# locuslab/lcp-physics

Hardware: NVIDIA H100
Metric: LCP solves/sec (LCPFunction fwd+bwd, batch=4096 x 64 contacts, fp32) (higher is better)
Workload: dtype f32 I/O and iterates; the condensed n x n KKT matrix is formed, factored and solved in f64

## Files before the change

### lcp_physics_b200/csrc/lcp_cond_kernels.cu

```cuda
#include "lcp_cond_launch.h"

namespace lcpb200 {
namespace cnd {

template <>
cudaError_t launch_cond_forward_t<LCP_T, LCP_NS>(const CFwdArgs<LCP_T>& a, int grid, cudaStream_t st) {
  if (a.prof) cond_forward_kernel<LCP_T, LCP_NS, true><<<grid, NT, a.P.smem_bytes, st>>>(a);
  else cond_forward_kernel<LCP_T, LCP_NS, false><<<grid, NT, a.P.smem_bytes, st>>>(a);
  return cudaGetLastError();
}

template <>
cudaError_t launch_cond_backward_t<LCP_T, LCP_NS>(const CBwdArgs<LCP_T>& a, int grid, cudaStream_t st) {
  if (a.prof) cond_backward_kernel<LCP_T, LCP_NS, true><<<grid, NT, a.P.smem_bytes, st>>>(a);
  else cond_backward_kernel<LCP_T, LCP_NS, false><<<grid, NT, a.P.smem_bytes, st>>>(a);
  return cudaGetLastError();
}

template <>
cudaError_t configure_cond_t<LCP_T, LCP_NS>(int smem_bytes, int dyn_max, int* occ) {
  cudaError_t e;
  const void* fns[4] = {(const void*)cond_forward_kernel<LCP_T, LCP_NS, false>, (const void*)cond_backward_kernel<LCP_T, LCP_NS, false>,
                        (const void*)cond_forward_kernel<LCP_T, LCP_NS, true>, (const void*)cond_backward_kernel<LCP_T, LCP_NS, true>};
  for (const void* f : fns)
    if ((e = cudaFuncSetAttribute(f, cudaFuncAttributeMaxDynamicSharedMemorySize, dyn_max)) != cudaSuccess) return e;
  int of = 0, ob = 0;
  if ((e = cudaOccupancyMaxActiveBlocksPerMultiprocessor(&of, fns[0], NT, smem_bytes)) != cudaSuccess) return e;
  if ((e = cudaOccupancyMaxActiveBlocksPerMultiprocessor(&ob, fns[1], NT, smem_bytes)) != cudaSuccess) return e;
  *occ = of < ob ? of : ob;
  return cudaSuccess;
}

}
}
```

### lcp_physics_b200/csrc/lcp_cond_launch.h

```cpp
#pragma once
#include <cuda_runtime.h>
#include "lcp_condensed.cuh"

namespace lcpb200 {
namespace cnd {

template <typename T, int NS> cudaError_t launch_cond_forward_t(const CFwdArgs<T>& a, int grid, cudaStream_t st);
template <typename T, int NS> cudaError_t launch_cond_backward_t(const CBwdArgs<T>& a, int grid, cudaStream_t st);
template <typename T, int NS> cudaError_t configure_cond_t(int smem_bytes, int dyn_max, int* occ);

}
}
```

### lcp_physics_b200/csrc/lcp_condensed.cuh

```cuda
#pragma once
#include "lcp_device.cuh"

namespace lcpb200 {
namespace cnd {

constexpr int NT = 256;
constexpr int UC = 8;
constexpr int CSMAX = 6;
constexpr int KS = 8;
constexpr int LMAX = 16;
constexpr int LU_BW = 2;
constexpr int MISC_BAND_LU = 4;
constexpr int CFLAG_DENSE_LU = 4;
constexpr int STATUS_UNSUPPORTED = -100;

struct CPlan {
  int ok;
  int n, m, e, N, NP, NS;
  int pcap;
  int wcap;
  int smem_bytes;
  int ctas_per_sm;
  int flags;
  int sbytes;
  int o_K, o_W, o_scr, o_bx, o_rdiag, o_Fd, o_Gd, o_As, o_x, o_rx, o_dx, o_qd, o_y, o_ry, o_dy,
      o_s, o_z, o_d, o_rz, o_ds, o_dz, o_rs2, o_red, o_rows, o_posof, o_clist, o_ccols, o_ncols, o_clcnt, o_misc;
};

__host__ __device__ inline size_t al16(size_t x) { return (x + 15) & ~(size_t)15; }
__host__ __device__ inline size_t scratch_bytes(int n, int m, int tsize) {
  return al16((size_t)2 * KS * m * 2) + al16((size_t)2 * KS * m * tsize) + al16((size_t)5 * m * 4) +
         al16((size_t)CSMAX * m * 2) + al16((size_t)8 * m * 4) + al16((size_t)LMAX * n * 2) + al16((size_t)n * 4) + 64;
}

inline size_t carve_plan(CPlan& P, int tsize) {
  size_t o = 0;
  const int n = P.n, m = P.m, e = P.e, NP = P.NP, pcap = P.pcap, wcap = P.wcap;
#define CND_TAKE(field, bytes) do { P.field = (int)o; o += al16((size_t)(bytes)); } while (0)
  size_t kb = (size_t)NP * NP * 8;
  if (scratch_bytes(n, m, tsize) > kb) kb = scratch_bytes(n, m, tsize);
  if ((size_t)8 * NP * 8 > kb) kb = (size_t)8 * NP * 8;
  { const size_t qn = (NP + 31) / 32, sl = (size_t)(NP / qn) * qn * qn * 32 * 8; if (sl > kb) kb = sl; }
  CND_TAKE(o_K, kb);
  CND_TAKE(o_W, (size_t)wcap * 8);
  CND_TAKE(o_scr, (size_t)pcap * 8);
  CND_TAKE(o_bx, (size_t)NP * 8);
  CND_TAKE(o_rdiag, (size_t)NP * 8);
  CND_TAKE(o_Fd, (size_t)wcap * tsize);
  CND_TAKE(o_Gd, (size_t)UC * pcap * tsize);
  CND_TAKE(o_As, (size_t)e * n * tsize);
  CND_TAKE(o_x, n * tsize); CND_TAKE(o_rx, n * tsize); CND_TAKE(o_dx, n * tsize); CND_TAKE(o_qd, n * tsize);
  CND_TAKE(o_y, e * tsize); CND_TAKE(o_ry, e * tsize); CND_TAKE(o_dy, e * tsize);
  CND_TAKE(o_s, m * tsize); CND_TAKE(o_z, m * tsize); CND_TAKE(o_d, m * tsize); CND_TAKE(o_rz, m * tsize);
  CND_TAKE(o_ds, m * tsize); CND_TAKE(o_dz, m * tsize); CND_TAKE(o_rs2, m * tsize);
  CND_TAKE(o_red, 192 * tsize);
  CND_TAKE(o_rows, pcap * 2);
  CND_TAKE(o_posof, m * 2);
  CND_TAKE(o_clist, LMAX * n * 2);
  CND_TAKE(o_ccols, UC * pcap);
  CND_TAKE(o_ncols, pcap);
  CND_TAKE(o_clcnt, n);
  CND_TAKE(o_misc, 16 * 4);
#undef CND_TAKE
  P.sbytes = 16 + (P.o_x - P.o_Fd) + (P.o_y - P.o_qd) + (P.o_misc - P.o_rows);
  return o;
}

extern __shared__ __align__(16) unsigned char cnd_smem[];

template <typename T>
struct CSmem {
  const CPlan& P;
  __device__ __forceinline__ explicit CSmem(const CPlan& p) : P(p) {}
#define CND_ACC(name, type) __device__ __forceinline__ type* name() const { return reinterpret_cast<type*>(cnd_smem + P.o_##name); }
  CND_ACC(K, double) CND_ACC(W, double) CND_ACC(scr, double) CND_ACC(bx, double) CND_ACC(rdiag, double)
  CND_ACC(Fd, T) CND_ACC(Gd, T) CND_ACC(As, T)
  CND_ACC(x, T) CND_ACC(rx, T) CND_ACC(dx, T) CND_ACC(qd, T) CND_ACC(y, T) CND_ACC(ry, T) CND_ACC(dy, T)
  CND_ACC(s, T) CND_ACC(z, T) CND_ACC(d, T) CND_ACC(rz, T) CND_ACC(ds, T) CND_ACC(dz, T) CND_ACC(rs2, T)
  CND_ACC(red, T)
  CND_ACC(rows, unsigned short) CND_ACC(posof, unsigned short) CND_ACC(clist, unsigned short)
  CND_ACC(ccols, unsigned char) CND_ACC(ncols, unsigned char) CND_ACC(clcnt, unsigned char)
  CND_ACC(misc, int)
#undef CND_ACC
};

struct Struct {
  int ncomp, cs;
  int sh;
  int m;
};

enum { CPH_STRUCT = 0, CPH_WINV, CPH_ASSEMBLE, CPH_LU, CPH_SOLVE_RHS, CPH_SOLVE_TRI, CPH_SOLVE_POST, CPH_RESID,
       CPH_STEP, CPH_GRADS, CPH_COUNT };
template <bool ON>
struct Prof {
  long long* p;
  long long t;
  __device__ __forceinline__ explicit Prof(long long* p_) : p(p_), t(0) {}
  __device__ __forceinline__ void start() { if (threadIdx.x == 0) t = clock64(); }
  __device__ __forceinline__ void lap(int ph) {
    if (threadIdx.x == 0) {
      const long long n = clock64();
      atomicAdd(reinterpret_cast<unsigned long long*>(p + ph), (unsigned long long)(n - t));
      t = n;
    }
  }
};
template <>
struct Prof<false> {
  __device__ __forceinline__ explicit Prof(long long*) {}
  __device__ __forceinline__ void start() {}
  __device__ __forceinline__ void lap(int) {}
};

template <typename T>
__device__ __forceinline__ int scan_rows(const T* __restrict__ A, int rows, int cols, T* vals, unsigned short* idx,
                                         int* cnt) {
  constexpr int CH = 8, RP = (sizeof(T) == 8) ? 2 : 4;
  const int lane = threadIdx.x & 31, warp = threadIdx.x >> 5, nw = NT >> 5;
  int bad = 0;
  if (cols <= 32 * CH) {
    for (int r0 = warp * RP; r0 < rows; r0 += nw * RP) {
      T v[RP][CH];
#pragma unroll
      for (int rr = 0; rr < RP; ++rr) {
        const T* row = A + (size_t)min(r0 + rr, rows - 1) * cols;
#pragma unroll
        for (int q = 0; q < CH; ++q) { const int j = q * 32 + lane; v[rr][q] = j < cols ? row[j] : T(0); }
      }
#pragma unroll
      for (int rr = 0; rr < RP; ++rr) {
        const int r = r0 + rr;
        if (r >= rows) break;
        int c = 0;
#pragma unroll
        for (int q = 0; q < CH; ++q) {
          const bool nz = v[rr][q] != T(0);
          const unsigned mask = __ballot_sync(FULL, nz);
          const int pos = c + __popc(mask & ((1u << lane) - 1u));
          if (nz && pos < KS) { vals[pos * rows + r] = v[rr][q]; idx[pos * rows + r] = (unsigned short)(q * 32 + lane); }
          c += __popc(mask);
        }
        if (c > KS) bad = 1;
        if (lane == 0) cnt[r] = c;
      }
    }
    return bad;
  }
  for (int r = warp; r < rows; r += nw) {
    const T* row = A + (size_t)r * cols;
    int c = 0;
    for (int j0 = 0; j0 < cols; j0 += 32 * CH) {
      T v[CH];
#pragma unroll
      for (int q = 0; q < CH; ++q) { const int j = j0 + q * 32 + lane; v[q] = j < cols ? row[j] : T(0); }
#pragma unroll
      for (int q = 0; q < CH; ++q) {
        const bool nz = v[q] != T(0);
        const unsigned mask = __ballot_sync(FULL, nz);
        const int pos = c + __popc(mask & ((1u << lane) - 1u));
        if (nz && pos < KS) { vals[pos * rows + r] = v[q]; idx[pos * rows + r] = (unsigned short)(j0 + q * 32 + lane); }
        c += __popc(mask);
      }
    }
    if (c > KS) bad = 1;
    if (lane == 0) cnt[r] = c;
  }
  return bad;
}

__device__ __forceinline__ void prefetch_l2(const void* p, size_t bytes) {
  const char* c = reinterpret_cast<const char*>(p);
  for (size_t o = (size_t)threadIdx.x * 128; o < bytes; o += (size_t)NT * 128)
    asm volatile("prefetch.global.L2 [%0];" ::"l"(c + o));
}

template <typename T>
__device__ __noinline__ bool build_structure(const CPlan& P, CSmem<T>& S, Struct& st, const T* __restrict__ Q,
                                             const T* __restrict__ G, const T* __restrict__ A,
                                             const T* __restrict__ F, int* singular) {
  const int n = P.n, m = P.m, e = P.e, tid = threadIdx.x, lane = tid & 31, warp = tid >> 5, pcap = P.pcap;
  prefetch_l2(F, (size_t)m * m * sizeof(T));
  prefetch_l2(G, (size_t)m * n * sizeof(T));
  prefetch_l2(Q, (size_t)n * n * sizeof(T));
  char* sb = reinterpret_cast<char*>(S.K());
  unsigned short* Fi = reinterpret_cast<unsigned short*>(sb);
  unsigned short* Gi = Fi + (size_t)KS * m;
  size_t o = al16((size_t)2 * KS * m * 2);
  T* Fv = reinterpret_cast<T*>(sb + o);
  T* Gv = Fv + (size_t)KS * m;
  o += al16((size_t)2 * KS * m * sizeof(T));
  int* Fcnt = reinterpret_cast<int*>(sb + o);
  int* Gcnt = Fcnt + m;
  int* label = Gcnt + m;
  int* cidx = label + m;
  int* memcnt = cidx + m;
  o += al16((size_t)5 * m * 4);
  unsigned short* memb = reinterpret_cast<unsigned short*>(sb + o);
  o += al16((size_t)CSMAX * m * 2);
  unsigned* cmap = reinterpret_cast<unsigned*>(sb + o);
  o += al16((size_t)8 * m * 4);
  unsigned short* cl_tmp = reinterpret_cast<unsigned short*>(sb + o);
  o += al16((size_t)LMAX * n * 2);
  int* cl_cnt = reinterpret_cast<int*>(sb + o);
  int* flags = S.misc();

  if (tid < 16) flags[tid] = 0;
  int bad = 0;
  for (int t = tid; t < n * n; t += NT) {
    const int i = t / n, j = t - i * n;
    const T q = Q[t];
    if (i == j) {
      S.qd()[i] = q;
      if (!(q != T(0) && isfinite((double)q))) bad |= 2;
    } else if (q != T(0)) bad |= 1;
  }
  bad |= scan_rows<T>(F, m, m, Fv, Fi, Fcnt) ? 1 : 0;
  bad |= scan_rows<T>(G, m, n, Gv, Gi, Gcnt) ? 1 : 0;
  for (int t = tid; t < e * n; t += NT) S.As()[t] = A[t];
  for (int i = tid; i < m; i += NT) { label[i] = i; memcnt[i] = 0; }
  for (int a = tid; a < n; a += NT) cl_cnt[a] = 0;
  const int anybad = __syncthreads_or(bad);
  if (anybad & 2) { *singular = 1; return false; }
  if (anybad & 1) return false;

  for (int pass = 0; pass < 64; ++pass) {
    int changed = 0;
    for (int i = tid; i < m; i += NT) {
      const int c = Fcnt[i];
      int li = ((volatile int*)label)[i];
      for (int k = 0; k < c; ++k) {
        const int j = Fi[k * m + i];
        const int lj = ((volatile int*)label)[j];
        if (lj < li) { li = lj; changed = 1; }
        else if (li < lj) { atomicMin(&label[j], li); changed = 1; }
      }
      atomicMin(&label[i], li);
    }
    if (!__syncthreads_or(changed)) break;
    if (pass == 63) return false;
  }
  if (m > 4 * NT) return false;
  int running = 0;
  for (int base = 0; base < m; base += NT) {
    const int i = base + tid;
    const bool root = i < m && label[i] == i;
    const unsigned mask = __ballot_sync(FULL, root);
    if (lane == 0) flags[8 + warp] = __popc(mask);
    __syncthreads();
    int before = running;
    for (int w = 0; w < warp; ++w) before += flags[8 + w];
    int total = 0;
    for (int w = 0; w < (NT >> 5); ++w) total += flags[8 + w];
    if (root) cidx[i] = before + __popc(mask & ((1u << lane) - 1u));
    if (i < m) {
      const int l = label[i];
      const int slot = atomicAdd(&memcnt[l], 1);
      if (slot < CSMAX) memb[l * CSMAX + slot] = (unsigned short)i;
    }
    running += total;
    __syncthreads();
  }
  const int ncomp = running;
  {
    int mx = 0;
    for (int i = tid; i < m; i += NT) mx = max(mx, memcnt[i]);
    if (mx > 0) atomicMax(&flags[3], mx);
  }
  __syncthreads();
  const int cs = flags[3];
  if (cs > CSMAX || ncomp * cs > pcap || ncomp * cs * cs > P.wcap || ncomp > 8191) return false;
  st.ncomp = ncomp; st.cs = cs; st.m = m;
  st.sh = 0;
  while ((1 << st.sh) < ncomp) ++st.sh;
  const int npos = ncomp * cs;
  for (int p = tid; p < npos; p += NT) { S.rows()[p] = 0xFFFF; S.ncols()[p] = 0; }
  for (int t = tid; t < ncomp * cs * cs; t += NT) S.Fd()[t] = T(0);
  for (int t = tid; t < UC * pcap; t += NT) { S.Gd()[t] = T(0); S.ccols()[t] = 0; }
  for (int t = tid; t < 8 * ncomp; t += NT) cmap[t] = 0u;
  __syncthreads();
  for (int i = tid; i < m; i += NT) {
    const int l = label[i], c = cidx[l], cnt = memcnt[l];
    int r = 0;
    for (int t = 0; t < cnt; ++t) r += (memb[l * CSMAX + t] < i);
    const int pos = r * ncomp + c;
    S.rows()[pos] = (unsigned short)i;
    S.posof()[i] = (unsigned short)pos;
    const int gc = Gcnt[i];
    for (int k = 0; k < gc; ++k) { const int col = Gi[k * m + i]; atomicOr(&cmap[c * 8 + (col >> 5)], 1u << (col & 31)); }
  }
  __syncthreads();
  int bad2 = 0;
  for (int i = tid; i < m; i += NT) {
    const int pos = S.posof()[i], r = pos / ncomp, c = pos - r * ncomp;
    const int fc = Fcnt[i];
    for (int k = 0; k < fc; ++k) {
      const int pj = S.posof()[Fi[k * m + i]];
      S.Fd()[(size_t)(r * cs + pj / ncomp) * ncomp + c] = Fv[k * m + i];
    }
    const int gc = Gcnt[i];
    for (int k = 0; k < gc; ++k) {
      const int col = Gi[k * m + i], wd = col >> 5;
      int p = __popc(cmap[c * 8 + wd] & ((1u << (col & 31)) - 1u));
      for (int w = 0; w < wd; ++w) p += __popc(cmap[c * 8 + w]);
      if (p < UC) { S.Gd()[(size_t)p * pcap + pos] = Gv[k * m + i]; S.ccols()[p * pcap + c] = (unsigned char)col; }
    }
  }
  for (int c = tid; c < ncomp; c += NT) {
    int cnt = 0;
#pragma unroll
    for (int w = 0; w < 8; ++w) cnt += __popc(cmap[c * 8 + w]);
    if (cnt > UC) bad2 = 1;
    S.ncols()[c] = (unsigned char)min(cnt, UC);
  }
  if (__syncthreads_or(bad2)) return false;
  int bad3 = 0;
  for (int t = tid; t < ncomp * UC; t += NT) {
    const int c = t / UC, p = t - c * UC;
    if (p < S.ncols()[c]) {
      const int a = S.ccols()[p * pcap + c];
      const int slot = atomicAdd(&cl_cnt[a], 1);
      if (slot < LMAX) cl_tmp[slot * n + a] = (unsigned short)(c * 8 + p); else bad3 = 1;
    }
  }
  if (__syncthreads_or(bad3)) return false;
  for (int t = tid; t < n * LMAX; t += NT) {
    const int a = t % n, l = t / n, cnt = cl_cnt[a];
    if (l < cnt) {
      const int v = cl_tmp[l * n + a];
      int rank = 0;
      for (int u = 0; u < cnt; ++u) rank += (cl_tmp[u * n + a] < v);
      S.clist()[rank * n + a] = (unsigned short)v;
    }
    if (l == 0) S.clcnt()[a] = (unsigned char)cnt;
  }
  __syncthreads();
  return true;
}

template <typename T>
struct EngineSoA {
  const T *mass, *inertia, *v, *fext;
  const T *normal, *p1, *p2;
  const T *mu, *rest;
  const int32_t *b1, *b2;
  const int32_t* nc_s;
  int nb, nc;
  int mode;
  T dt;
  T *p_s, *h_s;
};

template <typename T>
__device__ __forceinline__ void contact_row(T p1x, T p1y, T p2x, T p2y, T dx, T dy, T (&r1)[3], T (&r2)[3]) {
  r1[0] = p1x * dy - p1y * dx; r1[1] = dx; r1[2] = dy;
  r2[0] = -(p2x * dy - p2y * dx); r2[1] = -dx; r2[2] = -dy;
}

template <typename T>
__device__ __noinline__ bool build_structure_soa(const CPlan& P, CSmem<T>& S, Struct& st, const EngineSoA<T>& e_,
                                                 int sc, const T* __restrict__ A, int* singular) {
  const int n = P.n, e = P.e, tid = threadIdx.x, pcap = P.pcap;
  const int nb = e_.nb, ncs = e_.nc, cs = e_.mode == 0 ? 4 : 1;
  const int nc = e_.nc_s ? e_.nc_s[sc] : e_.nc;
  const int m = cs * nc;
  const int32_t* tb1 = e_.b1 + (e_.nc_s ? (size_t)sc * ncs : 0);
  const int32_t* tb2 = e_.b2 + (e_.nc_s ? (size_t)sc * ncs : 0);
  char* sb = reinterpret_cast<char*>(S.K());
  unsigned short* cl_tmp = reinterpret_cast<unsigned short*>(sb);
  int* cl_cnt = reinterpret_cast<int*>(sb + al16((size_t)LMAX * n * 2));
  if (n != 3 * nb || nc < 0 || nc > ncs || m > P.m || nc * cs > pcap || nc * cs * cs > P.wcap) return false;
  const T* mass = e_.mass + (size_t)sc * nb;
  const T* inertia = e_.inertia + (size_t)sc * nb;
  const T* v = e_.v + (size_t)sc * n;
  const T* normal = e_.normal + (size_t)sc * ncs * 2;
  const T* p1 = e_.p1 + (size_t)sc * ncs * 2;
  const T* p2 = e_.p2 + (size_t)sc * ncs * 2;
  T* ps = e_.p_s + (size_t)sc * n;
  T* hs = e_.h_s + (size_t)sc * P.m;
  int bad = 0;
  for (int j = tid; j < n; j += NT) {
    const int body = j / 3;
    const T q = (j - 3 * body == 0) ? inertia[body] : mass[body];
    S.qd()[j] = q;
    if (!(q != T(0) && isfinite((double)q))) bad |= 2;
    ps[j] = e_.mode == 0 ? q * v[j] + e_.dt * e_.fext[(size_t)sc * n + j] : T(0);
    cl_cnt[j] = 0;
  }
  for (int t = tid; t < e * n; t += NT) S.As()[t] = A[t];
  st.ncomp = nc; st.cs = cs; st.m = m;
  st.sh = 0;
  while ((1 << st.sh) < nc) ++st.sh;
  for (int t = tid; t < UC * pcap; t += NT) { S.Gd()[t] = T(0); S.ccols()[t] = 0; }
  for (int t = tid; t < nc * cs * cs; t += NT) S.Fd()[t] = T(0);
  __syncthreads();
  for (int c = tid; c < nc; c += NT) {
    const int b1 = tb1[c], b2 = tb2[c];
    if (b1 == b2 || b1 < 0 || b2 < 0 || b1 >= nb || b2 >= nb) { bad |= 1; continue; }
    const int lo = min(b1, b2), hi = max(b1, b2);
    const int o1 = b1 < b2 ? 0 : 3, o2 = 3 - o1;
#pragma unroll
    for (int q = 0; q < 3; ++q) {
      S.ccols()[q * pcap + c] = (unsigned char)(3 * lo + q);
      S.ccols()[(3 + q) * pcap + c] = (unsigned char)(3 * hi + q);
    }
    S.ncols()[c] = 6;
    const T nx = normal[2 * c], ny = normal[2 * c + 1];
    const T p1x = p1[2 * c], p1y = p1[2 * c + 1], p2x = p2[2 * c], p2y = p2[2 * c + 1];
    T r1[3], r2[3];
    contact_row<T>(p1x, p1y, p2x, p2y, nx, ny, r1, r2);
    const T jv = r1[0] * v[3 * b1] + r1[1] * v[3 * b1 + 1] + r1[2] * v[3 * b1 + 2] +
                 r2[0] * v[3 * b2] + r2[1] * v[3 * b2 + 1] + r2[2] * v[3 * b2 + 2];
    const T rc = e_.rest[(size_t)sc * ncs + c];
#pragma unroll
    for (int q = 0; q < 3; ++q) { S.Gd()[(size_t)(o1 + q) * pcap + c] = r1[q]; S.Gd()[(size_t)(o2 + q) * pcap + c] = r2[q]; }
    S.rows()[c] = (unsigned short)c;
    S.posof()[c] = (unsigned short)c;
    if (e_.mode == 0) {
      hs[c] = jv * rc;
      contact_row<T>(p1x, p1y, p2x, p2y, ny, -nx, r1, r2);
#pragma unroll
      for (int q = 0; q < 3; ++q) {
        S.Gd()[(size_t)(o1 + q) * pcap + nc + c] = r1[q];      S.Gd()[(size_t)(o2 + q) * pcap + nc + c] = r2[q];
        S.Gd()[(size_t)(o1 + q) * pcap + 2 * nc + c] = -r1[q]; S.Gd()[(size_t)(o2 + q) * pcap + 2 * nc + c] = -r2[q];
      }
      const int rw[4] = {c, nc + 2 * c, nc + 2 * c + 1, 3 * nc + c};
#pragma unroll
      for (int r = 0; r < 4; ++r) { S.rows()[r * nc + c] = (unsigned short)rw[r]; S.posof()[rw[r]] = (unsigned short)(r * nc + c); }
      hs[nc + 2 * c] = T(0); hs[nc + 2 * c + 1] = T(0); hs[3 * nc + c] = T(0);
      S.Fd()[(size_t)(1 * 4 + 3) * nc + c] = T(1);
      S.Fd()[(size_t)(2 * 4 + 3) * nc + c] = T(1);
      S.Fd()[(size_t)(3 * 4 + 0) * nc + c] = e_.mu[(size_t)sc * ncs + c];
      S.Fd()[(size_t)(3 * 4 + 1) * nc + c] = T(-1);
      S.Fd()[(size_t)(3 * 4 + 2) * nc + c] = T(-1);
    } else {
      hs[c] = jv + jv * -rc;
    }
    for (int q = 0; q < 6; ++q) {
      const int a = q < 3 ? 3 * lo + q : 3 * hi + q - 3;
      const int slot = atomicAdd(&cl_cnt[a], 1);
      if (slot < LMAX) cl_tmp[slot * n + a] = (unsigned short)(c * 8 + q); else bad |= 1;
    }
  }
  const int anybad = __syncthreads_or(bad);
  if (anybad & 2) { *singular = 1; return false; }
  if (anybad & 1) return false;
  for (int t = tid; t < n * LMAX; t += NT) {
    const int a = t % n, l = t / n, cnt = cl_cnt[a];
    if (l < cnt) {
      const int val = cl_tmp[l * n + a];
      int rank = 0;
      for (int u = 0; u < cnt; ++u) rank += (cl_tmp[u * n + a] < val);
      S.clist()[rank * n + a] = (unsigned short)val;
    }
    if (l == 0) S.clcnt()[a] = (unsigned char)cnt;
  }
  __syncthreads();
  return true;
}

template <typename T>
__device__ __noinline__ void mark_band_lu(const CPlan& P, CSmem<T> S, Struct st) {
  int wide = P.e > 0 || (P.flags & CFLAG_DENSE_LU);
  for (int c = threadIdx.x; c < st.ncomp; c += NT) {
    const int nc = S.ncols()[c];
    if (nc > 0 && (S.ccols()[(nc - 1) * P.pcap + c] >> 4) - (S.ccols()[c] >> 4) > LU_BW) wide = 1;
  }
  wide = __syncthreads_or(wide);
  if (threadIdx.x == 0) S.misc()[MISC_BAND_LU] = !wide;
}

__device__ __forceinline__ double rcp64_fast(double x) {
  double r;
  asm("rcp.approx.ftz.f64 %0, %1;" : "=d"(r) : "d"(x));
  const double ax = fabs(x);
  if (!(ax > 1e-290 && ax < 1e290)) return 1.0 / x;
  r = fma(r, fma(-x, r, 1.0), r);
  r = fma(r, fma(-x, r, 1.0), r);
  return r;
}

template <typename T, int CS>
__device__ __forceinline__ void comp_inverse(const CPlan& P, CSmem<T>& S, const Struct& st) {
  const int nc_ = st.ncomp;
  for (int c = threadIdx.x; c < nc_; c += NT) {
    double M[CS][CS];
#pragma unroll
    for (int r = 0; r < CS; ++r) {
      const int i = S.rows()[r * nc_ + c];
#pragma unroll
      for (int q = 0; q < CS; ++q) M[r][q] = (double)S.Fd()[(size_t)(r * CS + q) * nc_ + c];
      M[r][r] += (i == 0xFFFF) ? 1.0 : ((P.flags & 1) ? 1.0 / (double)S.d()[i] : (double)(T(1) / S.d()[i]));
    }
    unsigned swaps = 0;
    int bit = 0;
#pragma unroll
    for (int k = 0; k < CS; ++k) {
#pragma unroll
      for (int i = k + 1; i < CS; ++i) {
        const bool sw = fabs(M[i][k]) > fabs(M[k][k]);
        swaps |= (sw ? 1u : 0u) << bit;
        ++bit;
#pragma unroll
        for (int q = 0; q < CS; ++q) { const double u = M[k][q], w = M[i][q]; M[k][q] = sw ? w : u; M[i][q] = sw ? u : w; }
      }
      const double r = rcp64_fast(M[k][k]);
      M[k][k] = 1.0;
#pragma unroll
      for (int q = 0; q < CS; ++q) M[k][q] *= r;
#pragma unroll
      for (int i = 0; i < CS; ++i) {
        if (i == k) continue;
        const double f = M[i][k];
        M[i][k] = 0.0;
#pragma unroll
        for (int q = 0; q < CS; ++q) M[i][q] = fma(-f, M[k][q], M[i][q]);
      }
    }
#pragma unroll
    for (int k = CS - 1; k >= 0; --k) {
#pragma unroll
      for (int i = CS - 1; i > k; --i) {
        --bit;
        const bool sw = (swaps >> bit) & 1u;
#pragma unroll
        for (int q = 0; q < CS; ++q) { const double u = M[q][k], w = M[q][i]; M[q][k] = sw ? w : u; M[q][i] = sw ? u : w; }
      }
    }
#pragma unroll
    for (int r = 0; r < CS; ++r)
#pragma unroll
      for (int q = 0; q < CS; ++q) S.W()[(size_t)(r * CS + q) * nc_ + c] = M[r][q];
  }
}

template <typename T, int CS>
__device__ __forceinline__ void comp_apply(CSmem<T>& S, const Struct& st, bool trans = false) {
  const int nc_ = st.ncomp;
  const int npos = nc_ * CS;
  const int sh = st.sh, cmask = (1 << sh) - 1, tot = CS << sh;
  double val[4];
#pragma unroll
  for (int u = 0; u < 4; ++u) {
    const int t = threadIdx.x + u * NT, r = t >> sh, c = t & cmask;
    val[u] = 0.0;
    if (t < tot && c < nc_) {
      double a = 0.0;
#pragma unroll
      for (int q = 0; q < CS; ++q) a = fma(S.W()[(size_t)(trans ? (q * CS + r) : (r * CS + q)) * nc_ + c], S.scr()[q * nc_ + c], a);
      val[u] = a;
    }
  }
  __syncthreads();
#pragma unroll
  for (int u = 0; u < 4; ++u) {
    const int t = threadIdx.x + u * NT, r = t >> sh, c = t & cmask;
    if (t < tot && c < nc_) S.scr()[r * nc_ + c] = val[u];
  }
  (void)npos;
}

template <typename T, int NS, int CS>
__device__ __forceinline__ void assemble_K(const CPlan& P, CSmem<T>& S, const Struct& st) {
  const int nc_ = st.ncomp;
  constexpr int NP = 16 * NS;
  const int n = P.n, N = P.N, e = P.e, tid = threadIdx.x, pcap = P.pcap;
  double* K = S.K();
  {
    double2* K2 = reinterpret_cast<double2*>(K);
    for (int t = tid; t < NP * NP / 2; t += NT) K2[t] = make_double2(0.0, 0.0);
  }
  __syncthreads();
  for (int i = tid; i < NP; i += NT) K[(size_t)i * NP + i] = i < n ? (double)S.qd()[i] : (i < N ? 0.0 : 1.0);
  for (int t = tid; t < e * n; t += NT) {
    const int k = t / n, i = t - k * n;
    const double v = (double)S.As()[t];
    K[(size_t)(n + k) * NP + i] = v;
    K[(size_t)i * NP + n + k] = v;
  }
  __syncthreads();
  const int grp = tid >> 3, q2 = tid & 7;
  for (int a0 = 0; a0 < n; a0 += NT / 8) {
    const int a = a0 + grp;
    const int cnt = a < n ? (int)S.clcnt()[a] : 0;
    int mx = cnt;
    mx = max(mx, __shfl_xor_sync(FULL, mx, 8));
    mx = max(mx, __shfl_xor_sync(FULL, mx, 16));
    for (int l = 0; l < mx; ++l) {
      if (l < cnt) {
        const int cp = S.clist()[l * n + a], c = cp >> 3, p = cp & 7;
        if (q2 < (int)S.ncols()[c]) {
          double acc = 0.0;
#pragma unroll
          for (int q = 0; q < CS; ++q) {
            double u = 0.0;
#pragma unroll
            for (int r = 0; r < CS; ++r)
              u = fma((double)S.Gd()[(size_t)p * pcap + r * nc_ + c], S.W()[(size_t)(r * CS + q) * nc_ + c], u);
            acc = fma(u, (double)S.Gd()[(size_t)q2 * pcap + q * nc_ + c], acc);
          }
          K[(size_t)S.ccols()[q2 * pcap + c] * NP + a] += acc;
        }
      }
      __syncwarp();
    }
  }
  __syncthreads();
}

template <int NS, int BW>
struct LuBand {
  static constexpr bool DENSE = BW >= NS - 1;
  static constexpr int W = DENSE ? NS : 2 * BW + 1;
  static __device__ __forceinline__ constexpr bool in(int r, int c) { return DENSE || (r - c <= BW && c - r <= BW); }
  static __device__ __forceinline__ constexpr int col(int r, int c) { return DENSE ? c : c - r + BW; }
  static __host__ __device__ constexpr int end(int b0) { return DENSE || b0 + BW + 1 > NS ? NS : b0 + BW + 1; }
};

template <int NS, int BW, int B0>
__device__ __forceinline__ void lu_phase(double (&a)[NS][LuBand<NS, BW>::W], int o_buf, int o_rdiag, int& step, int ti,
                                         int tj) {
  using Bd = LuBand<NS, BW>;
  constexpr int NP = 16 * NS;
  constexpr int E = Bd::end(B0);
  constexpr int L = E - B0;
  constexpr int CW = (L <= 4) ? L : 3;
  double* const rdiag = reinterpret_cast<double*>(cnd_smem + o_rdiag);
#pragma unroll 1
  for (int kk = 0; kk < 16; kk += 2) {
    const int k = 16 * B0 + kk;
    double2* const U2 = reinterpret_cast<double2*>(cnd_smem + o_buf) + (size_t)(step & 1) * 2 * NP;
    double2* const C2 = U2 + NP;
    ++step;
    {
      const int sr = ti - kk, sc = tj - kk;
      if ((unsigned)sr < 2u) {
        double* dst = reinterpret_cast<double*>(U2) + sr;
#pragma unroll
        for (int c = B0; c < E; ++c) dst[2 * (16 * c + tj)] = a[B0][Bd::col(B0, c)];
      }
      if ((unsigned)sc < 2u) {
        double* dst = reinterpret_cast<double*>(C2) + sc;
#pragma unroll
        for (int r = B0; r < E; ++r) dst[2 * (16 * r + ti)] = a[r][Bd::col(r, B0)];
      }
    }
    __syncthreads();
    const double2 pk = U2[k], pk1 = U2[k + 1];
    const double p01 = pk1.x;
    const double r0 = rcp64_fast(pk.x);
    const double r1 = pk.x * rcp64_fast(fma(pk.x, pk1.y, -(pk.y * p01)));
    const double l10 = pk.y * r0;
    if ((ti | tj) == 0) { rdiag[k] = r0; rdiag[k + 1] = r1; }
#pragma unroll
    for (int cg = B0; cg < E; cg += CW) {
      double w0[CW], w1[CW];
#pragma unroll
      for (int q = 0; q < CW; ++q) {
        const int c = cg + q;
        if (c < E) {
          const double2 u = U2[16 * c + tj];
          const double x1 = fma(-l10, u.x, u.y);
          w0[q] = (c == B0 && !(tj > kk)) ? 0.0 : u.x;
          w1[q] = (c == B0 && !(tj > kk + 1)) ? 0.0 : x1;
        }
      }
#pragma unroll
      for (int r = B0; r < E; ++r) {
        const double2 cc = C2[16 * r + ti];
        double m0 = cc.x * r0;
        double m1 = fma(-m0, p01, cc.y) * r1;
        if (r == B0) {
          m0 = (ti > kk) ? m0 : 0.0;
          m1 = (ti > kk + 1) ? m1 : 0.0;
        }
#pragma unroll
        for (int q = 0; q < CW; ++q) {
          const int c = cg + q;
          if (c < E) a[r][Bd::col(r, c)] = fma(-m1, w1[q], fma(-m0, w0[q], a[r][Bd::col(r, c)]));
        }
      }
    }
  }
}

template <int NS, int BW, int B0>
struct LuPhases {
  static __device__ __forceinline__ void run(double (&a)[NS][LuBand<NS, BW>::W], int o_buf, int o_rdiag, int& step, int ti,
                                             int tj) {
    lu_phase<NS, BW, B0>(a, o_buf, o_rdiag, step, ti, tj);
    LuPhases<NS, BW, B0 + 1>::run(a, o_buf, o_rdiag, step, ti, tj);
  }
};
template <int NS, int BW>
struct LuPhases<NS, BW, NS> {
  static __device__ __forceinline__ void run(double (&)[NS][LuBand<NS, BW>::W], int, int, int&, int, int) {}
};

template <int NS> struct SolveLayout {
  static constexpr int NP = 16 * NS;
  static constexpr int QN = (NP + 31) / 32;
  static constexpr int ROUNDS = NP / QN;
  static constexpr size_t BYTES = (size_t)ROUNDS * QN * QN * 32 * 8;
};

template <int NS, int BW>
__device__ __forceinline__ void factor_K_body(int o_K, int o_rdiag, bool trans) {
  using Bd = LuBand<NS, BW>;
  constexpr int NP = 16 * NS, QN = SolveLayout<NS>::QN;
  int tid_;
  asm volatile("mov.u32 %0, %%tid.x;" : "=r"(tid_));
  const int ti = tid_ & 15, tj = tid_ >> 4;
  double* const K = reinterpret_cast<double*>(cnd_smem + o_K);
  double* const rdiag = reinterpret_cast<double*>(cnd_smem + o_rdiag);
  double a[NS][Bd::W];
#pragma unroll
  for (int c = 0; c < NS; ++c)
#pragma unroll
    for (int r = 0; r < NS; ++r)
      if (Bd::in(r, c)) a[r][Bd::col(r, c)] = K[(size_t)(16 * c + tj) * NP + 16 * r + ti];
  __syncthreads();
  int step = 0;
  LuPhases<NS, BW, 0>::run(a, o_K, o_rdiag, step, ti, tj);
  __syncthreads();
  int rowpart[NS];
  double rrow[NS];
#pragma unroll
  for (int r = 0; r < NS; ++r) {
    const int i = 16 * r + ti;
    rowpart[r] = trans ? (i / QN) * QN * QN * 32 + (i % QN) * 32 : (i % QN) * QN * 32 + i / QN;
    rrow[r] = rdiag[i];
  }
#pragma unroll
  for (int c = 0; c < NS; ++c) {
    const int j = 16 * c + tj;
    const double rj = rdiag[j];
    const int colpart = trans ? (j % QN) * QN * 32 + j / QN : (j / QN) * QN * QN * 32 + (j % QN) * 32;
#pragma unroll
    for (int r = 0; r < NS; ++r) {
      const int i = 16 * r + ti;
      const double v = Bd::in(r, c) ? a[r][Bd::col(r, c)] : 0.0;
      K[colpart + rowpart[r]] = (i != j) ? v * (trans ? rrow[r] : rj) : v;
    }
  }
  __syncthreads();
}

template <int NS>
__device__ __noinline__ void factor_K(int o_K, int o_rdiag, bool trans, bool band) {
  if constexpr (LU_BW < NS - 1) {
    if (band) {
      factor_K_body<NS, LU_BW>(o_K, o_rdiag, trans);
      return;
    }
  }
  factor_K_body<NS, NS - 1>(o_K, o_rdiag, trans);
}

template <int QN>
struct SolveCoef {
  double dg[QN * QN];
  double rw[QN * QN];
};

template <int QN>
__device__ __forceinline__ void solve_load(SolveCoef<QN>& c, const double* blk, int r, int lane) {
#pragma unroll
  for (int t = 0; t < QN * QN; ++t) { c.dg[t] = blk[t * 32 + r]; c.rw[t] = blk[t * 32 + lane]; }
}

template <int QN>
__device__ __forceinline__ void solve_round_fwd(double (&y)[QN], const SolveCoef<QN>& c, int r, int lane) {
  double v[QN];
#pragma unroll
  for (int q = 0; q < QN; ++q) v[q] = __shfl_sync(FULL, y[q], r);
#pragma unroll
  for (int q = 0; q < QN; ++q)
#pragma unroll
    for (int qp = q + 1; qp < QN; ++qp) v[qp] = fma(-c.dg[qp * QN + q], v[q], v[qp]);
  const bool below = lane > r, own = lane == r;
#pragma unroll
  for (int qp = 0; qp < QN; ++qp) {
    double t = y[qp];
#pragma unroll
    for (int q = 0; q < QN; ++q) t = fma(-c.rw[qp * QN + q], v[q], t);
    y[qp] = below ? t : (own ? v[qp] : y[qp]);
  }
}

template <int QN>
__device__ __forceinline__ void solve_round_bwd(double (&y)[QN], const SolveCoef<QN>& c, int r, int lane) {
  double v[QN];
#pragma unroll
  for (int q = 0; q < QN; ++q) v[q] = __shfl_sync(FULL, y[q], r);
#pragma unroll
  for (int q = QN - 1; q >= 0; --q)
#pragma unroll
    for (int qp = q - 1; qp >= 0; --qp) v[qp] = fma(-c.dg[qp * QN + q], v[q], v[qp]);
  const bool above = lane < r, own = lane == r;
#pragma unroll
  for (int qp = 0; qp < QN; ++qp) {
    double t = y[qp];
#pragma unroll
    for (int q = QN - 1; q >= 0; --q) t = fma(-c.rw[qp * QN + q], v[q], t);
    y[qp] = above ? t : (own ? v[qp] : y[qp]);
  }
}

template <int NS>
__device__ __noinline__ void solve_warp(int o_K, int o_rdiag, int o_bx) {
  constexpr int NP = 16 * NS, QN = SolveLayout<NS>::QN, ROUNDS = SolveLayout<NS>::ROUNDS;
  constexpr int STRIDE = QN * QN * 32;
  static_assert(ROUNDS % 2 == 0, "the software pipeline handles two rounds per trip");
  const int lane = threadIdx.x & 31;
  const double* const S = reinterpret_cast<const double*>(cnd_smem + o_K);
  const double* const rdiag = reinterpret_cast<const double*>(cnd_smem + o_rdiag);
  double* const bx = reinterpret_cast<double*>(cnd_smem + o_bx);
  double y[QN];
#pragma unroll
  for (int q = 0; q < QN; ++q) y[q] = (QN * lane + q < NP) ? bx[QN * lane + q] : 0.0;
  SolveCoef<QN> c0, c1;
  solve_load<QN>(c0, S, 0, lane);
#pragma unroll 1
  for (int r = 0; r < ROUNDS; r += 2) {
    solve_load<QN>(c1, S + (size_t)(r + 1) * STRIDE, r + 1, lane);
    solve_round_fwd<QN>(y, c0, r, lane);
    const int rn = (r + 2 < ROUNDS) ? r + 2 : ROUNDS - 1;
    solve_load<QN>(c0, S + (size_t)rn * STRIDE, rn, lane);
    solve_round_fwd<QN>(y, c1, r + 1, lane);
  }
#pragma unroll 1
  for (int r = ROUNDS - 1; r > 0; r -= 2) {
    solve_load<QN>(c1, S + (size_t)(r - 1) * STRIDE, r - 1, lane);
    solve_round_bwd<QN>(y, c0, r, lane);
    const int rn = (r - 2 >= 0) ? r - 2 : 0;
    solve_load<QN>(c0, S + (size_t)rn * STRIDE, rn, lane);
    solve_round_bwd<QN>(y, c1, r - 1, lane);
  }
#pragma unroll
  for (int q = 0; q < QN; ++q) {
    const int i = QN * lane + q;
    if (i < NP) bx[i] = y[q] * rdiag[i];
  }
}

template <typename T, int CS, int NS, typename PF>
__device__ __noinline__ void solve_kkt(const CPlan& P, CSmem<T> S, Struct st, PF& pf, const T* rx,
                                       const T* rs, const T* rz, const T* ry, T* dx, T* ds, T* dz, T* dy,
                                       bool trans = false) {
  const int nc_ = st.ncomp;
  const int n = P.n, e = P.e, N = P.N, NP = P.NP, tid = threadIdx.x, pcap = P.pcap;
  const int npos = st.ncomp * CS;
  for (int p = tid; p < npos; p += NT) {
    const int i = S.rows()[p];
    double t = 0.0;
    if (i != 0xFFFF) t = (P.flags & 2) ? ((double)(rz ? rz[i] : T(0)) - (double)rs[i] / (double)S.d()[i]) : (double)((rz ? rz[i] : T(0)) - rs[i] / S.d()[i]);
    S.scr()[p] = t;
  }
  __syncthreads();
  comp_apply<T, CS>(S, st, trans);
  __syncthreads();
  for (int a = tid; a < NP; a += NT) {
    double acc = 0.0;
    if (a < n) {
      const int cnt = S.clcnt()[a];
      for (int l = 0; l < cnt; ++l) {
        const int cp = S.clist()[l * n + a], c = cp >> 3, p = cp & 7;
#pragma unroll
        for (int r = 0; r < CS; ++r) acc = fma((double)S.Gd()[(size_t)p * pcap + r * nc_ + c], S.scr()[r * nc_ + c], acc);
      }
      acc = -(double)(rx ? rx[a] : T(0)) - acc;
    } else if (a < N) {
      acc = -(double)(ry ? ry[a - n] : T(0));
    }
    S.bx()[a] = acc;
  }
  __syncthreads();
  pf.lap(CPH_SOLVE_RHS);
  if (tid < 32) solve_warp<NS>(P.o_K, P.o_rdiag, P.o_bx);
  __syncthreads();
  pf.lap(CPH_SOLVE_TRI);
  for (int tt = tid; tt < (CS << st.sh); tt += NT) {
    const int c = tt & ((1 << st.sh) - 1);
    if (c >= nc_) continue;
    const int p = (tt >> st.sh) * nc_ + c;
    const int i = S.rows()[p];
    double t = 0.0;
    if (i != 0xFFFF) {
      const int nc = S.ncols()[c];
      t = (P.flags & 2) ? ((double)(rz ? rz[i] : T(0)) - (double)rs[i] / (double)S.d()[i]) : (double)((rz ? rz[i] : T(0)) - rs[i] / S.d()[i]);
      for (int q = 0; q < nc; ++q) t = fma((double)S.Gd()[(size_t)q * pcap + p], S.bx()[S.ccols()[q * pcap + c]], t);
    }
    S.scr()[p] = t;
  }
  __syncthreads();
  comp_apply<T, CS>(S, st, trans);
  __syncthreads();
  for (int p = tid; p < npos; p += NT) {
    const int i = S.rows()[p];
    if (i == 0xFFFF) continue;
    const T wz = (T)S.scr()[p];
    const T rsi = rs[i];
    dz[i] = wz;
    ds[i] = (-rsi - wz) / S.d()[i];
  }
  for (int a = tid; a < n; a += NT) dx[a] = (T)S.bx()[a];
  for (int k = tid; k < e; k += NT) dy[k] = (T)S.bx()[n + k];
  __syncthreads();
  pf.lap(CPH_SOLVE_POST);
}

template <typename T, int NS, int CS, typename PF>
__device__ __noinline__ void factor_kkt(const CPlan& P, CSmem<T> S, Struct st, PF& pf, bool trans = false) {
  comp_inverse<T, CS>(P, S, st);
  __syncthreads();
  pf.lap(CPH_WINV);
  assemble_K<T, NS, CS>(P, S, st);
  pf.lap(CPH_ASSEMBLE);
  if constexpr (LU_BW < NS - 1) factor_K<NS>(P.o_K, P.o_rdiag, trans, S.misc()[MISC_BAND_LU] != 0);
  else factor_K<NS>(P.o_K, P.o_rdiag, trans, false);
  pf.lap(CPH_LU);
}

template <typename T>
__device__ __forceinline__ void get_steps(const T* z, const T* dz, const T* s, const T* ds, int m, T* red, T& step_z,
                                          T& step_s) {
  const T NEG_INF = -INFINITY, POS_INF = INFINITY;
  T mx[2] = {NEG_INF, NEG_INF};
  T mn[2] = {POS_INF, POS_INF};
  T any[2] = {T(0), T(0)};
  for (int i = threadIdx.x; i < m; i += NT) {
    const T az = -z[i] / dz[i], as = -s[i] / ds[i];
    mx[0] = nan_max(mx[0], az);
    mx[1] = nan_max(mx[1], as);
    if (dz[i] > T(0)) any[0] = T(1); else mn[0] = nan_min(mn[0], az);
    if (ds[i] > T(0)) any[1] = T(1); else mn[1] = nan_min(mn[1], as);
  }
  T v[6] = {mx[0], mx[1], -mn[0], -mn[1], any[0], any[1]};
  block_reduce<T, 6>(v, OpMax(), NEG_INF, red);
  const T fz = (v[0] > T(1)) ? v[0] : T(1);
  const T fs = (v[1] > T(1)) ? v[1] : T(1);
  step_z = (v[4] > T(0)) ? nan_min(-v[2], fz) : -v[2];
  step_s = (v[5] > T(0)) ? nan_min(-v[3], fs) : -v[3];
}

template <typename T>
struct CFwdArgs {
  CPlan P;
  int B;
  const T *Q, *p, *G, *h, *A, *b, *F;
  T *zhat, *nu, *lam, *slack, *resid;
  int *status, *iters;
  T eps;
  int not_improved_lim, max_iter;
  long long* prof;
  EngineSoA<T> soa;
  unsigned char* ssave;
};

template <typename T>
struct CBwdArgs {
  CPlan P;
  int B;
  const T *Q, *G, *A, *F;
  const T *zhat, *nu, *lam, *slack, *g;
  T *dQ, *dp, *dG, *dh, *dA, *db, *dF;
  int* done;
  const int* only;
  unsigned flags;
  const unsigned char* sload;
  EngineSoA<T> soa;
  T *dmass, *dinertia, *dv, *dfext, *dnormal, *dp1, *dp2, *dmu, *drest;
  long long* prof;
};

__device__ __forceinline__ void copy16(unsigned char* dst, const unsigned char* src, int bytes) {
  const uint4* s4 = reinterpret_cast<const uint4*>(src);
  uint4* d4 = reinterpret_cast<uint4*>(dst);
  for (int i = threadIdx.x; i < (bytes >> 4); i += NT) d4[i] = s4[i];
}

__device__ __forceinline__ void save_structure(const CPlan& P, const Struct& st, bool ok, unsigned char* dst) {
  if (threadIdx.x == 0) *reinterpret_cast<int4*>(dst) = make_int4(ok ? st.ncomp : -1, st.cs, st.sh, st.m);
  if (!ok) return;
  const int c1 = P.o_x - P.o_Fd, c2 = P.o_y - P.o_qd, c3 = P.o_misc - P.o_rows;
  copy16(dst + 16, cnd_smem + P.o_Fd, c1);
  copy16(dst + 16 + c1, cnd_smem + P.o_qd, c2);
  copy16(dst + 16 + c1 + c2, cnd_smem + P.o_rows, c3);
}

__device__ __forceinline__ bool load_structure(const CPlan& P, Struct& st, const unsigned char* src) {
  const int4 hd = *reinterpret_cast<const int4*>(src);
  st.ncomp = hd.x; st.cs = hd.y; st.sh = hd.z; st.m = hd.w;
  if (hd.x < 0) return false;
  const int c1 = P.o_x - P.o_Fd, c2 = P.o_y - P.o_qd, c3 = P.o_misc - P.o_rows;
  copy16(cnd_smem + P.o_Fd, src + 16, c1);
  copy16(cnd_smem + P.o_qd, src + 16 + c1, c2);
  copy16(cnd_smem + P.o_rows, src + 16 + c1 + c2, c3);
  return true;
}

template <typename T>
struct SzResid { T sz, resid; };

template <typename T, int CS>
__device__ __noinline__ SzResid<T> fwd_residuals(const CFwdArgs<T>& a, CSmem<T> S, Struct st, int sc) {
  const int nc_ = st.ncomp;
  const CPlan& P = a.P;
  const int n = P.n, m = st.m, e = P.e, tid = threadIdx.x, pcap = P.pcap;
  const T* p = a.p + (size_t)sc * n;
  const T* h = a.h + (size_t)sc * P.m;
  const T* b = e > 0 ? a.b + (size_t)sc * e : nullptr;
  for (int c = tid; c < n; c += NT) {
    T acc = 0;
    const int cnt = S.clcnt()[c];
    for (int l = 0; l < cnt; ++l) {
      const int cp = S.clist()[l * n + c], cc = cp >> 3, pp = cp & 7;
#pragma unroll
      for (int r = 0; r < CS; ++r) {
        const int i = S.rows()[r * nc_ + cc];
        if (i != 0xFFFF) acc = fma(S.Gd()[(size_t)pp * pcap + r * nc_ + cc], S.z()[i], acc);
      }
    }
    for (int k = 0; k < e; ++k) acc = fma(S.As()[k * n + c], S.y()[k], acc);
    S.rx()[c] = acc + S.qd()[c] * S.x()[c] + p[c];
  }
  for (int tt = tid; tt < (CS << st.sh); tt += NT) {
    const int r = tt >> st.sh, c = tt & ((1 << st.sh) - 1);
    if (c >= nc_) continue;
    const int pz = r * nc_ + c;
    const int i = S.rows()[pz];
    if (i == 0xFFFF) continue;
    const int nc = S.ncols()[c];
    T acc = 0;
    for (int q = 0; q < nc; ++q) acc = fma(S.Gd()[(size_t)q * pcap + pz], S.x()[S.ccols()[q * pcap + c]], acc);
    T fz = 0;
#pragma unroll
    for (int q = 0; q < CS; ++q) {
      const int j = S.rows()[q * nc_ + c];
      if (j != 0xFFFF) fz = fma(S.Fd()[(size_t)(r * CS + q) * nc_ + c], S.z()[j], fz);
    }
    S.rz()[i] = acc + S.s()[i] - h[i] - fz;
  }
  for (int k = tid; k < e; k += NT) {
    T acc = 0;
    for (int j = 0; j < n; ++j) acc = fma(S.As()[k * n + j], S.x()[j], acc);
    S.ry()[k] = acc - b[k];
  }
  __syncthreads();
  T q4[4] = {0, 0, 0, 0};
  for (int i = tid; i < m; i += NT) { q4[0] += S.s()[i] * S.z()[i]; q4[1] += S.rz()[i] * S.rz()[i]; }
  for (int i = tid; i < e; i += NT) q4[2] += S.ry()[i] * S.ry()[i];
  for (int i = tid; i < n; i += NT) q4[3] += S.rx()[i] * S.rx()[i];
  block_reduce<T, 4>(q4, OpSum(), T(0), S.red());
  const T sz = q4[0];
  const T mu = fabs(sz / T(m));
  return {sz, (e > 0 ? sqrt(q4[2]) : T(0)) + sqrt(q4[1]) + sqrt(q4[3]) + T(m) * mu};
}

template <typename T>
__device__ __noinline__ void fwd_store_best(const CFwdArgs<T>& a, CSmem<T> S, int m, int sc) {
  const CPlan& P = a.P;
  const int n = P.n, e = P.e, tid = threadIdx.x;
  for (int i = tid; i < n; i += NT) a.zhat[(size_t)sc * n + i] = S.x()[i];
  for (int i = tid; i < m; i += NT) { a.lam[(size_t)sc * P.m + i] = S.z()[i]; a.slack[(size_t)sc * P.m + i] = S.s()[i]; }
  for (int i = tid; i < e; i += NT) a.nu[(size_t)sc * e + i] = S.y()[i];
}

template <typename T>
__device__ __noinline__ void fwd_centering(CSmem<T> S, int m, T mu, T sz) {
  const int tid = threadIdx.x;
  T stz, sts;
  get_steps(S.z(), S.dz(), S.s(), S.ds(), m, S.red(), stz, sts);
  const T alpha_aff = nan_min(nan_min(stz, sts), T(1));
  T t3[1] = {0};
  for (int i = tid; i < m; i += NT) t3[0] += (S.s()[i] + alpha_aff * S.ds()[i]) * (S.z()[i] + alpha_aff * S.dz()[i]);
  block_reduce<T, 1>(t3, OpSum(), T(0), S.red());
  const T ratio = t3[0] / sz;
  const T sig = ratio * ratio * ratio;
  const T musig = -mu * sig;
  for (int i = tid; i < m; i += NT) S.rs2()[i] = (musig + S.ds()[i] * S.dz()[i]) / S.s()[i];
  __syncthreads();
}

template <typename T>
__device__ __noinline__ void fwd_step(const CPlan& P, CSmem<T> S, int m) {
  const int n = P.n, e = P.e, tid = threadIdx.x;
  for (int i = tid; i < n; i += NT) S.dx()[i] += S.rx()[i];
  for (int i = tid; i < m; i += NT) { S.ds()[i] += S.rz()[i]; S.dz()[i] += S.rs2()[i]; }
  for (int i = tid; i < e; i += NT) S.dy()[i] += S.ry()[i];
  __syncthreads();
  T stz, sts;
  get_steps(S.z(), S.dz(), S.s(), S.ds(), m, S.red(), stz, sts);
  const T alpha = nan_min(T(0.999) * nan_min(stz, sts), T(1));
  for (int i = tid; i < n; i += NT) S.x()[i] += alpha * S.dx()[i];
  for (int i = tid; i < m; i += NT) { S.s()[i] += alpha * S.ds()[i]; S.z()[i] += alpha * S.dz()[i]; }
  for (int i = tid; i < e; i += NT) S.y()[i] += alpha * S.dy()[i];
  __syncthreads();
}

template <typename T, int NS, int CS, typename PF>
__device__ __forceinline__ void forward_scene(const CFwdArgs<T>& a, CSmem<T>& S, const Struct& st, PF& pf, int sc) {
  const CPlan& P = a.P;
  const int m = st.m;
  {
    const int n = P.n, e = P.e, tid = threadIdx.x;
    const T* h = a.h + (size_t)sc * P.m;
    const T* b = e > 0 ? a.b + (size_t)sc * e : nullptr;
    for (int i = tid; i < m; i += NT) { S.d()[i] = T(1); S.rs2()[i] = T(0); S.rz()[i] = -h[i]; }
    for (int i = tid; i < n; i += NT) S.rx()[i] = a.p[(size_t)sc * n + i];
    for (int i = tid; i < e; i += NT) S.ry()[i] = -b[i];
    __syncthreads();
  }
  factor_kkt<T, NS, CS>(P, S, st, pf);
  solve_kkt<T, CS, NS>(P, S, st, pf, S.rx(), S.rs2(), S.rz(), P.e > 0 ? S.ry() : nullptr, S.x(), S.s(), S.z(), S.y());
  if (m == 0) {
    fwd_store_best<T>(a, S, 0, sc);
    if (threadIdx.x == 0) { a.status[sc] = 2; a.iters[sc] = 0; if (a.resid) a.resid[sc] = T(0); }
    return;
  }
  {
    const int tid = threadIdx.x;
    T mn[2] = {INFINITY, INFINITY};
    for (int i = tid; i < m; i += NT) { mn[0] = nan_min(mn[0], S.s()[i]); mn[1] = nan_min(mn[1], S.z()[i]); }
    block_reduce<T, 2>(mn, OpMin(), (T)INFINITY, S.red());
    for (int i = tid; i < m; i += NT) {
      if (mn[0] <= T(0)) S.s()[i] -= mn[0] - T(1);
      if (mn[1] <= T(0)) S.z()[i] -= mn[1] - T(1);
    }
    __syncthreads();
  }

  T best = nan("");
  bool have_best = false;
  int not_improved = 0, status = 0, it = 0;
  for (it = 0; it < a.max_iter; ++it) {
    const SzResid<T> r = fwd_residuals<T, CS>(a, S, st, sc);
    pf.lap(CPH_RESID);
    const T mu = fabs(r.sz / T(m));

    bool improved;
    if (!have_best) { improved = true; have_best = true; not_improved = 0; }
    else { improved = r.resid < best; not_improved = improved ? 0 : not_improved + 1; }
    if (improved) {
      best = r.resid;
      fwd_store_best<T>(a, S, m, sc);
    }
    if (not_improved == a.not_improved_lim) { status = 1; ++it; break; }
    if (best < a.eps) { status = 2; ++it; break; }
    if (mu > T(1e100)) { status = 3; ++it; break; }

    for (int i = threadIdx.x; i < m; i += NT) S.d()[i] = S.z()[i] / S.s()[i];
    __syncthreads();
    factor_kkt<T, NS, CS>(P, S, st, pf);

    solve_kkt<T, CS, NS>(P, S, st, pf, S.rx(), S.z(), S.rz(), P.e > 0 ? S.ry() : nullptr, S.dx(), S.ds(), S.dz(), S.dy());
    fwd_centering<T>(S, m, mu, r.sz);
    pf.lap(CPH_STEP);
    solve_kkt<T, CS, NS>(P, S, st, pf, nullptr, S.rs2(), nullptr, nullptr, S.rx(), S.rz(), S.rs2(), S.ry());
    fwd_step<T>(P, S, m);
    pf.lap(CPH_STEP);
  }
  if (threadIdx.x == 0) { a.status[sc] = status; a.iters[sc] = it; if (a.resid) a.resid[sc] = best; }
}

template <typename T, int NS, bool PROF>
__global__ void __launch_bounds__(NT, (NS <= 6) ? 2 : 1) cond_forward_kernel(const __grid_constant__ CFwdArgs<T> a) {
  const CPlan& P = a.P;
  CSmem<T> S(P);
  const int n = P.n, m = P.m, e = P.e, tid = threadIdx.x;
  __shared__ int singular_s;
  const T NANV = nan("");
  Prof<PROF> pf(PROF ? a.prof + (size_t)blockIdx.x * CPH_COUNT : nullptr);
  for (int sc = blockIdx.x; sc < a.B; sc += gridDim.x) {
    if (tid == 0) singular_s = 0;
    __syncthreads();
    pf.start();
    Struct st;
    const bool ok = a.soa.mass
        ? build_structure_soa<T>(P, S, st, a.soa, sc, e > 0 ? a.A + (size_t)sc * e * n : nullptr, &singular_s)
        : build_structure<T>(P, S, st, a.Q + (size_t)sc * n * n, a.G + (size_t)sc * m * n,
                             e > 0 ? a.A + (size_t)sc * e * n : nullptr, a.F + (size_t)sc * m * m, &singular_s);
    __syncthreads();
    if (a.ssave) save_structure(P, st, ok, a.ssave + (size_t)sc * P.sbytes);
    pf.lap(CPH_STRUCT);
    if (!ok) {
      if (singular_s) {
        for (int i = tid; i < n; i += NT) a.zhat[(size_t)sc * n + i] = NANV;
        for (int i = tid; i < m; i += NT) { a.lam[(size_t)sc * m + i] = NANV; a.slack[(size_t)sc * m + i] = NANV; }
        for (int i = tid; i < e; i += NT) a.nu[(size_t)sc * e + i] = NANV;
        if (tid == 0) { a.status[sc] = -1; a.iters[sc] = 0; if (a.resid) a.resid[sc] = NANV; }
      } else if (tid == 0) {
        a.status[sc] = STATUS_UNSUPPORTED;
      }
      __syncthreads();
      continue;
    }
    if constexpr (LU_BW < NS - 1) mark_band_lu<T>(P, S, st);
    switch (st.cs) {
      case 1: forward_scene<T, NS, 1>(a, S, st, pf, sc); break;
      case 2: forward_scene<T, NS, 2>(a, S, st, pf, sc); break;
      case 3: forward_scene<T, NS, 3>(a, S, st, pf, sc); break;
      case 4: forward_scene<T, NS, 4>(a, S, st, pf, sc); break;
      case 5: forward_scene<T, NS, 5>(a, S, st, pf, sc); break;
      default: forward_scene<T, NS, 6>(a, S, st, pf, sc); break;
    }
    __syncthreads();
  }
}

template <typename T, typename F>
__device__ __forceinline__ void write_outer(T* __restrict__ o, int rows, int cols, F f) {
  constexpr int V = 16 / (int)sizeof(T);
  const int tid = threadIdx.x;
  if (cols % V == 0 && (reinterpret_cast<size_t>(o) & 15) == 0) {
    const int cv = cols / V, total = rows * cv;
    const int di = NT / cv, dj = NT - di * cv;
    int i = tid / cv, jv = tid - i * cv;
    for (int t = tid; t < total; t += NT) {
      const int j = jv * V;
      if (V == 4) {
        float4 w;
        w.x = (float)f(i, j); w.y = (float)f(i, j + 1); w.z = (float)f(i, j + 2); w.w = (float)f(i, j + 3);
        reinterpret_cast<float4*>(o)[t] = w;
      } else {
        double2 w;
        w.x = (double)f(i, j); w.y = (double)f(i, j + 1);
        reinterpret_cast<double2*>(o)[t] = w;
      }
      i += di; jv += dj;
      if (jv >= cv) { jv -= cv; ++i; }
    }
  } else {
    int i = tid / cols, j = tid - i * cols;
    const int di = NT / cols, dj = NT - di * cols;
    for (size_t t = tid; t < (size_t)rows * cols; t += NT) {
      o[t] = f(i, j);
      i += di; j += dj;
      if (j >= cols) { j -= cols; ++i; }
    }
  }
}

template <typename T, int NS, int CS, typename PF>
__device__ __forceinline__ void backward_scene(const CBwdArgs<T>& a, CSmem<T>& S, const Struct& st, PF& pf, int sc) {
  const CPlan& P = a.P;
  const int n = P.n, m = st.m, e = P.e, tid = threadIdx.x;
  const T* zh = a.zhat + (size_t)sc * n;
  const T* lam = a.lam + (size_t)sc * P.m;
  const T* slk = a.slack + (size_t)sc * P.m;
  const T* nu = e > 0 ? a.nu + (size_t)sc * e : nullptr;
  for (int i = tid; i < n; i += NT) { S.x()[i] = zh[i]; S.rx()[i] = a.g[(size_t)sc * n + i]; }
  for (int i = tid; i < m; i += NT) {
    T d = lam[i] / slk[i];
    if (sizeof(T) == 8) d = d > T(1e10) ? T(1e10) : (d < T(1e-10) ? T(1e-10) : d);
    S.z()[i] = lam[i]; S.s()[i] = slk[i]; S.d()[i] = d; S.rs2()[i] = T(0);
  }
  for (int i = tid; i < e; i += NT) S.y()[i] = nu[i];
  __syncthreads();
  const bool exact = (a.flags & 1u) != 0;
  factor_kkt<T, NS, CS>(P, S, st, pf, exact);
  solve_kkt<T, CS, NS>(P, S, st, pf, S.rx(), S.rs2(), nullptr, nullptr, S.dx(), S.ds(), S.dz(), S.dy(), exact);
  const T* dx = S.dx(); const T* dlam = S.dz(); const T* dnu = S.dy();
  if (a.soa.mass) {
    const EngineSoA<T>& E = a.soa;
    const int nc = st.ncomp, nb = E.nb, ncs = E.nc;
    const int32_t* tb1 = E.b1 + (E.nc_s ? (size_t)sc * ncs : 0);
    const int32_t* tb2 = E.b2 + (E.nc_s ? (size_t)sc * ncs : 0);
    const T* v = E.v + (size_t)sc * n;
    const T* zh_ = S.x(); const T* lm = S.z();
    for (int c = tid; c < ncs; c += NT) {
      const size_t ic = (size_t)sc * ncs + c;
      if (c >= nc) {
        if (a.dnormal) { a.dnormal[ic * 2] = 0; a.dnormal[ic * 2 + 1] = 0; }
        if (a.dp1) { a.dp1[ic * 2] = 0; a.dp1[ic * 2 + 1] = 0; }
        if (a.dp2) { a.dp2[ic * 2] = 0; a.dp2[ic * 2 + 1] = 0; }
        if (a.drest) a.drest[ic] = 0;
        if (a.dmu) a.dmu[ic] = 0;
        continue;
      }
      const T nx = E.normal[ic * 2], ny = E.normal[ic * 2 + 1];
      const T p1x = E.p1[ic * 2], p1y = E.p1[ic * 2 + 1], p2x = E.p2[ic * 2], p2y = E.p2[ic * 2 + 1];
      const int j1 = 3 * tb1[c], j2 = 3 * tb2[c];
      const T rc = E.rest[ic];
      const T dhc = -dlam[c] * (E.mode == 0 ? T(1) : T(1));
      T gnx = 0, gny = 0, g1x = 0, g1y = 0, g2x = 0, g2y = 0, jcv = 0;
      const int nrows = E.mode == 0 ? 3 : 1;
      const int rows_[3] = {c, nc + 2 * c, nc + 2 * c + 1};
      const T dxs[3] = {nx, ny, -ny}, dys[3] = {ny, -nx, nx};
      for (int q = 0; q < nrows; ++q) {
        const T ddx_ = dxs[q], ddy_ = dys[q];
        const int i = rows_[q];
        T g[6];
        for (int t = 0; t < 3; ++t) {
          g[t] = dlam[i] * zh_[j1 + t] + lm[i] * dx[j1 + t];
          g[3 + t] = dlam[i] * zh_[j2 + t] + lm[i] * dx[j2 + t];
        }
        if (q == 0) {
          const T row[6] = {p1x * ddy_ - p1y * ddx_, ddx_, ddy_, -(p2x * ddy_ - p2y * ddx_), -ddx_, -ddy_};
          for (int t = 0; t < 3; ++t) jcv += row[t] * v[j1 + t] + row[3 + t] * v[j2 + t];
          const T hs_ = E.mode == 0 ? rc : (T(1) - rc);
          for (int t = 0; t < 3; ++t) { g[t] += dhc * hs_ * v[j1 + t]; g[3 + t] += dhc * hs_ * v[j2 + t]; }
        }
        const T gdx = -p1y * g[0] + g[1] + p2y * g[3] - g[4];
        const T gdy = p1x * g[0] + g[2] - p2x * g[3] - g[5];
        g1x += ddy_ * g[0]; g1y += -ddx_ * g[0];
        g2x += -ddy_ * g[3]; g2y += ddx_ * g[3];
        if (q == 0) { gnx += gdx; gny += gdy; }
        else if (q == 1) { gny += gdx; gnx += -gdy; }
        else { gny += -gdx; gnx += gdy; }
      }
      if (a.dnormal) { a.dnormal[ic * 2] = gnx; a.dnormal[ic * 2 + 1] = gny; }
      if (a.dp1) { a.dp1[ic * 2] = g1x; a.dp1[ic * 2 + 1] = g1y; }
      if (a.dp2) { a.dp2[ic * 2] = g2x; a.dp2[ic * 2 + 1] = g2y; }
      if (a.drest) a.drest[ic] = E.mode == 0 ? dhc * jcv : -dhc * jcv;
      if (a.dmu) a.dmu[ic] = E.mode == 0 ? -(dlam[3 * nc + c] * lm[c]) : T(0);
    }
    for (int j = tid; j < n; j += NT) {
      const int body = j / 3, comp = j - 3 * body;
      const T md = comp == 0 ? E.inertia[(size_t)sc * nb + body] : E.mass[(size_t)sc * nb + body];
      const T dpj = E.mode == 0 ? dx[j] : T(0);
      if (a.dfext) a.dfext[(size_t)sc * n + j] = E.dt * dpj;
      if (a.dv) {
        T acc = md * dpj;
        const int cnt = S.clcnt()[j];
        for (int l = 0; l < cnt; ++l) {
          const int cp = S.clist()[l * n + j], c = cp >> 3, pslot = cp & 7;
          const T hs_ = E.mode == 0 ? E.rest[(size_t)sc * ncs + c] : (T(1) - E.rest[(size_t)sc * ncs + c]);
          acc += -dlam[c] * hs_ * S.Gd()[(size_t)pslot * P.pcap + c];
        }
        a.dv[(size_t)sc * n + j] = acc;
      }
      const T dqjj = dx[j] * zh_[j];
      if (comp == 0 && a.dinertia) a.dinertia[(size_t)sc * nb + body] = dqjj + dpj * v[j];
    }
    __syncthreads();
    for (int body = tid; body < nb; body += NT) {
      if (!a.dmass) break;
      T acc = 0;
      for (int comp = 1; comp < 3; ++comp) {
        const int j = 3 * body + comp;
        acc += dx[j] * zh_[j] + (E.mode == 0 ? dx[j] : T(0)) * v[j];
      }
      a.dmass[(size_t)sc * nb + body] = acc;
    }
    if (a.db && e > 0) for (int i = tid; i < e; i += NT) a.db[(size_t)sc * e + i] = -dnu[i];
    if (a.dA && e > 0) {
      T* o = a.dA + (size_t)sc * e * n;
      for (int i = 0; i < e; ++i)
        for (int j = tid; j < n; j += NT) o[(size_t)i * n + j] = dnu[i] * S.x()[j] + S.y()[i] * dx[j];
    }
    if (tid == 0 && a.done) a.done[sc] = 1;
    __syncthreads();
    pf.lap(CPH_GRADS);
    return;
  }
  if (a.dp) for (int i = tid; i < n; i += NT) a.dp[(size_t)sc * n + i] = dx[i];
  if (a.dh) for (int i = tid; i < m; i += NT) a.dh[(size_t)sc * m + i] = -dlam[i];
  if (a.db && e > 0) for (int i = tid; i < e; i += NT) a.db[(size_t)sc * e + i] = -dnu[i];
  if (a.dG)
    write_outer<T>(a.dG + (size_t)sc * m * n, m, n, [&](int i, int j) { return dlam[i] * S.x()[j] + S.z()[i] * dx[j]; });
  if (a.dF)
    write_outer<T>(a.dF + (size_t)sc * m * m, m, m, [&](int i, int j) { return -(dlam[i] * S.z()[j]); });
  if (a.dA && e > 0)
    write_outer<T>(a.dA + (size_t)sc * e * n, e, n, [&](int i, int j) { return dnu[i] * S.x()[j] + S.y()[i] * dx[j]; });
  if (a.dQ)
    write_outer<T>(a.dQ + (size_t)sc * n * n, n, n, [&](int i, int j) { return T(0.5) * (dx[i] * S.x()[j] + S.x()[i] * dx[j]); });
  if (tid == 0 && a.done) a.done[sc] = 1;
  __syncthreads();
  pf.lap(CPH_GRADS);
}

template <typename T, int NS, bool PROF>
__global__ void __launch_bounds__(NT, (NS <= 6) ? 2 : 1) cond_backward_kernel(const __grid_constant__ CBwdArgs<T> a) {
  const CPlan& P = a.P;
  CSmem<T> S(P);
  const int n = P.n, m = P.m, e = P.e, tid = threadIdx.x;
  __shared__ int singular_s;
  Prof<PROF> pf(PROF ? a.prof + (size_t)blockIdx.x * CPH_COUNT : nullptr);
  for (int sc = blockIdx.x; sc < a.B; sc += gridDim.x) {
    if (a.only && !a.only[sc]) continue;
    if (tid == 0) singular_s = 0;
    __syncthreads();
    pf.start();
    Struct st;
    const bool ok = a.soa.mass
        ? build_structure_soa<T>(P, S, st, a.soa, sc, e > 0 ? a.A + (size_t)sc * e * n : nullptr, &singular_s)
        : a.sload
              ? load_structure(P, st, a.sload + (size_t)sc * P.sbytes)
              : build_structure<T>(P, S, st, a.Q + (size_t)sc * n * n, a.G + (size_t)sc * m * n,
                                   e > 0 ? a.A + (size_t)sc * e * n : nullptr, a.F + (size_t)sc * m * m, &singular_s);
    __syncthreads();
    pf.lap(CPH_STRUCT);
    if (!ok) {
      if (tid == 0 && a.done) a.done[sc] = 0;
      __syncthreads();
      continue;
    }
    if constexpr (LU_BW < NS - 1) mark_band_lu<T>(P, S, st);
    switch (st.cs) {
      case 1: backward_scene<T, NS, 1>(a, S, st, pf, sc); break;
      case 2: backward_scene<T, NS, 2>(a, S, st, pf, sc); break;
      case 3: backward_scene<T, NS, 3>(a, S, st, pf, sc); break;
      case 4: backward_scene<T, NS, 4>(a, S, st, pf, sc); break;
      case 5: backward_scene<T, NS, 5>(a, S, st, pf, sc); break;
      default: backward_scene<T, NS, 6>(a, S, st, pf, sc); break;
    }
    __syncthreads();
  }
}

}
}
```

### lcp_physics_b200/csrc/lcpb200.cu

```cuda
#include <cuda_runtime.h>
#include <stdio.h>
#include <string.h>
#include <algorithm>
#include <new>
#include <string>
#include <vector>

#include "../../include/lcpb200.h"
#include "lcp_assemble.cuh"
#include "lcp_launch.h"
#include "lcp_cond_launch.h"
#include "lcp_band_launch.h"
#include "lcp_contacts.cuh"

using namespace lcpb200;
using cnd::CPlan;

static thread_local std::string g_err;
static int fail(const std::string& s) { g_err = s; return 1; }
#define CK(call)                                                                                 \
  do {                                                                                           \
    cudaError_t _e = (call);                                                                     \
    if (_e != cudaSuccess)                                                                       \
      return fail(std::string(#call) + ": " + cudaGetErrorString(_e) + " (" __FILE__ ":" +      \
                  std::to_string(__LINE__) + ")");                                               \
  } while (0)

struct DeviceGuard {
  int prev = -1;
  bool armed = false;
  cudaError_t set(int device) {
    cudaError_t e = cudaGetDevice(&prev);
    if (e != cudaSuccess) return e;
    armed = (prev != device);
    return armed ? cudaSetDevice(device) : cudaSuccess;
  }
  ~DeviceGuard() { if (armed) cudaSetDevice(prev); }
};

struct DevBuf {
  void* p = nullptr;
  size_t bytes = 0;
  cudaError_t ensure(size_t need) {
    if (need <= bytes) return cudaSuccess;
    if (p) cudaFree(p);
    p = nullptr; bytes = 0;
    cudaError_t e = cudaMalloc(&p, need);
    if (e == cudaSuccess) bytes = need;
    return e;
  }
  void release() { if (p) cudaFree(p); p = nullptr; bytes = 0; }
};

struct lcpb200_handle_s {
  int dtype, n, m, e, device;
  int num_sms, smem_optin;
  Plan plan;
  int max_grid;
  CPlan cplan;
  int cond_grid = 0;
  static const int NSLOT = 2;
  void* ws = nullptr;
  size_t ws_bytes = 0;
  int ws_ctas = 0;
  DevBuf d_flag[NSLOT];
  DevBuf d_ph;
  bool dual_ok = true;
  bnd::BPlan bplan;
  int bplan_mode = -1;
  DevBuf d_bwsd, d_bwsi;
  int bws_ctas = 0;
  cudaStream_t streams[NSLOT] = {nullptr, nullptr};
  DevBuf d_in[7], d_out[6], d_bwd[16];
  long long* prof = nullptr;
  long long* cprof = nullptr;
  DevBuf d_struct;
  int struct_B = 0;
  DevBuf d_R;
  int retained_B = 0;
  bool retained_R = false;
};

static int pad_ld(int cols, int elem_bytes) {
  const int wpe = elem_bytes / 4;
  int ld = cols;
  while ((ld * wpe) % 32 != 4 || (ld * elem_bytes) % 16 != 0) ++ld;
  return ld;
}

template <typename T>
static int make_plan(lcpb200_handle_s* h) {
  Plan& P = h->plan;
  const int n = h->n, m = h->m, e = h->e;
  constexpr int NB = Blk<T>::NB, VC = VecOf<T>::VC;
  const int w = (int)sizeof(T);
  memset(&P, 0, sizeof(P));
  P.n = n; P.m = m; P.e = e;
  P.mp = ((m + NB - 1) / NB) * NB;
  const int mp = P.mp;
  P.nt = (mp >= 96 || n >= 96) ? 512 : (mp >= 64 ? 256 : 128);
  Vecs<T> vv;
  P.lds = pad_ld(NB, w);
  const long long vec_elems = vv.carve(nullptr, n, mp, e, P.nt, NB, P.lds);
  long long budget = (long long)h->smem_optin - 1024 - vec_elems * w;
  if (budget < 0) return fail("problem too large: the shared-memory vectors alone exceed the per-CTA limit");
  auto al4 = [](long long x) { return (x + 3) & ~3LL; };
  long long off = 0;
  const int ldfull = pad_ld(mp, w);
  if ((long long)mp * ldfull * w <= budget) {
    P.mode = 0; P.m1 = mp; P.ldT = ldfull; P.ldL = 0;
    P.off_T = (int)off; off += al4((long long)mp * ldfull);
  } else {
    const int m1 = (((mp / 2) + NB - 1) / NB) * NB, n2 = mp - m1;
    const int ldl = pad_ld(m1, w);
    const int tiles = ((n2 + 15) / 16) * ((n2 + 16 * VC - 1) / (16 * VC));
    const long long need = ((long long)m1 * ldfull + (long long)n2 * ldl) * w;
    if (n2 > 0 && n2 <= m1 && need <= budget && tiles <= P.nt / 32) {
      P.mode = 1; P.m1 = m1; P.ldT = ldfull; P.ldL = ldl;
      P.off_T = (int)off; off += al4((long long)m1 * ldfull);
      P.off_L = (int)off; off += al4((long long)n2 * ldl);
    } else {
      P.mode = 2; P.m1 = mp; P.ldT = ((mp + VC - 1) / VC) * VC; P.ldL = 0;
    }
  }
  P.stage_ld = 0;
  P.prefetch = getenv("LCPB200_NO_PREFETCH") ? 0 : 1;
  if (P.mode != 2) {
    const int lds = pad_ld(n, w);
    if ((long long)m * lds <= (long long)P.m1 * P.ldT) P.stage_ld = lds;
  }
  budget -= off * w;
  P.ldG = n;
  P.ldQi = ((n + VC - 1) / VC) * VC;
  const long long Gb = al4((long long)m * P.ldG), Qb = al4((long long)n * P.ldQi);
  if (Gb * w <= budget) { P.G_smem = 1; P.off_G = (int)off; off += Gb; budget -= Gb * w; }
  if (Qb * w <= budget) { P.Qi_smem = 1; P.off_Qi = (int)off; off += Qb; budget -= Qb * w; }
  P.off_vec = (int)off;
  P.smem_bytes = (int)((off + vec_elems) * w);
  long long ws = 0;
  P.w_Qi = ws; ws += Qb;
  P.w_R = ws; ws += al4((long long)m * m);
  P.w_T = ws; ws += (P.mode == 2) ? al4((long long)mp * P.ldT) : 0;
  P.w_U12 = ws; ws += (P.mode == 1) ? al4((long long)P.m1 * (mp - P.m1)) : 0;
  P.w_X = ws; ws += al4((long long)n * m);
  P.w_XA = ws; ws += al4((long long)n * e);
  P.w_S11 = ws; ws += al4((long long)e * e);
  P.w_V = ws; ws += al4((long long)m * e);
  P.w_W = ws; ws += al4((long long)e * m);
  P.w_Fell = ws; ws += al4((long long)m * 8);
  P.w_Gell = ws; ws += al4((long long)16 * m + (long long)64 * n);
  P.ws_per_cta = ws;
  return 0;
}

template <typename T>
static int configure_kernels(lcpb200_handle_s* h) {
  const Plan& P = h->plan;
  const int dyn_max = h->smem_optin - 1024;
  int occ = 0;
  cudaError_t ce = P.mode == 0 ? configure_t<T, 0>(P.nt, P.smem_bytes, dyn_max, &occ)
                 : P.mode == 1 ? configure_t<T, 1>(P.nt, P.smem_bytes, dyn_max, &occ)
                               : configure_t<T, 2>(P.nt, P.smem_bytes, dyn_max, &occ);
  if (ce != cudaSuccess) return fail(std::string("kernel configuration: ") + cudaGetErrorString(ce));
  if (occ < 1) return fail("kernel cannot be resident with the planned shared memory");
  occ = std::min(occ, 8);
  h->max_grid = occ * h->num_sms;
  h->plan.grid = h->max_grid;
  return 0;
}


#define LCPB200_NS_DISPATCH(NSV, CALL)                                  \
  ((NSV) == 2 ? CALL(2) : (NSV) == 3 ? CALL(3) : (NSV) == 4 ? CALL(4) : (NSV) == 6 ? CALL(6) : CALL(8))

template <typename T>
static int make_cplan(lcpb200_handle_s* h) {
  CPlan& C = h->cplan;
  memset(&C, 0, sizeof(C));
  if (getenv("LCPB200_NO_CONDENSED")) return 0;
  const int n = h->n, m = h->m, e = h->e, N = n + e;
  if (N > 128 || n > 255 || m > 4 * cnd::NT) return 0;
  static const int sizes[5] = {2, 3, 4, 6, 8};
  int NS = 8;
  for (int k = 4; k >= 0; --k) if (16 * sizes[k] >= N) NS = sizes[k];
  C.n = n; C.m = m; C.e = e; C.N = N; C.NS = NS; C.NP = 16 * NS;
  C.pcap = (m + 7) & ~7;
  C.flags = getenv("LCPB200_COND_FLAGS") ? atoi(getenv("LCPB200_COND_FLAGS")) : 3;
  const int dyn_max = h->smem_optin - 1024;
  const int target = NS <= 6 ? 2 : 1;
  const int per_cta_target = (228 * 1024) / target - 1024 - 64;
  int best = -1;
  for (int want = target; want >= 1 && best < 0; --want) {
    const int lim = std::min(dyn_max, want == target ? per_cta_target : (228 * 1024) / want - 1024 - 64);
    for (int mult = cnd::CSMAX; mult >= 1; --mult) {
      C.wcap = mult * C.pcap;
      const size_t bytes = cnd::carve_plan(C, (int)sizeof(T));
      if ((long long)bytes <= lim) { best = (int)bytes; break; }
      if (mult <= 4) break;
    }
  }
  if (best < 0) return 0;
  C.smem_bytes = best;
  int occ = 0;
#define CALL_CFG(NSV) cnd::configure_cond_t<T, NSV>(C.smem_bytes, dyn_max, &occ)
  const cudaError_t ce = LCPB200_NS_DISPATCH(NS, CALL_CFG);
#undef CALL_CFG
  if (ce != cudaSuccess) return fail(std::string("condensed kernel configuration: ") + cudaGetErrorString(ce));
  if (occ < 1) return 0;
  C.ctas_per_sm = occ;
  h->cond_grid = occ * h->num_sms;
  C.ok = 1;
  return 0;
}

extern "C" int lcpb200_version(void) { return LCPB200_VERSION; }
extern "C" const char* lcpb200_last_error_string(void) { return g_err.c_str(); }

extern "C" int lcpb200_create(int dtype, int n, int m, int e, int device, lcpb200_handle_t* out) {
  if (!out) return fail("out == NULL");
  *out = nullptr;
  if (dtype != LCPB200_F32 && dtype != LCPB200_F64) return fail("dtype must be LCPB200_F32 or LCPB200_F64");
  if (n <= 0 || m <= 0 || e < 0) return fail("need n > 0, m > 0, e >= 0");
  DeviceGuard dg_;
  CK(dg_.set(device));
  lcpb200_handle_s* h = new (std::nothrow) lcpb200_handle_s();
  if (!h) return fail("out of host memory");
  h->dtype = dtype; h->n = n; h->m = m; h->e = e; h->device = device;
  cudaError_t ce;
  if ((ce = cudaDeviceGetAttribute(&h->num_sms, cudaDevAttrMultiProcessorCount, device)) != cudaSuccess ||
      (ce = cudaDeviceGetAttribute(&h->smem_optin, cudaDevAttrMaxSharedMemoryPerBlockOptin, device)) != cudaSuccess) {
    delete h;
    return fail(std::string("cudaDeviceGetAttribute: ") + cudaGetErrorString(ce));
  }
  int rc = (dtype == LCPB200_F32) ? make_plan<float>(h) : make_plan<double>(h);
  if (!rc) rc = (dtype == LCPB200_F32) ? configure_kernels<float>(h) : configure_kernels<double>(h);
  if (rc) {
    if (dtype != LCPB200_F64 || n % 3 != 0 || e > bnd::BD) { delete h; return rc; }
    h->dual_ok = false;
    h->max_grid = h->num_sms;
    rc = 0;
  }
  if (!rc) rc = (dtype == LCPB200_F32) ? make_cplan<float>(h) : make_cplan<double>(h);
  if (rc) { delete h; return rc; }
  memset(&h->bplan, 0, sizeof(h->bplan));
  *out = h;
  return 0;
}

static int ensure_ws(lcpb200_handle_s* h, int B) {
  const int ctas = std::min(B, h->max_grid);
  if (ctas <= h->ws_ctas) return 0;
  const size_t esz = h->dtype == LCPB200_F32 ? 4 : 8;
  const size_t need = (size_t)h->plan.ws_per_cta * esz * (size_t)ctas * lcpb200_handle_s::NSLOT;
  if (h->ws) { CK(cudaDeviceSynchronize()); CK(cudaFree(h->ws)); h->ws = nullptr; h->ws_bytes = 0; h->ws_ctas = 0; }
  CK(cudaMalloc(&h->ws, need));
  h->ws_bytes = need;
  h->ws_ctas = ctas;
  return 0;
}

extern "C" int lcpb200_destroy(lcpb200_handle_t h) {
  if (!h) return 0;
  DeviceGuard dg_;
  dg_.set(h->device);
  if (h->ws) cudaFree(h->ws);
  h->d_struct.release();
  if (h->prof) cudaFree(h->prof);
  if (h->cprof) cudaFree(h->cprof);
  for (auto& s : h->streams) if (s) cudaStreamDestroy(s);
  for (auto& b : h->d_in) b.release();
  for (auto& b : h->d_out) b.release();
  for (auto& b : h->d_bwd) b.release();
  for (auto& b : h->d_flag) b.release();
  h->d_ph.release();
  h->d_bwsd.release();
  h->d_bwsi.release();
  h->d_R.release();
  delete h;
  return 0;
}

extern "C" size_t lcpb200_workspace_bytes(lcpb200_handle_t h) { return h ? h->ws_bytes : 0; }

extern "C" int lcpb200_describe(lcpb200_handle_t h, char* buf, size_t len) {
  if (!h || !buf) return fail("null argument");
  const Plan& P = h->plan;
  static const char* modes[3] = {"smem", "smem-split(U12 in L2)", "L2"};
  const CPlan& C = h->cplan;
  char cbuf[256];
  if (C.ok)
    snprintf(cbuf, sizeof(cbuf), "condensed KKT: N=%d(pad %d) fp64 LU in registers, threads=%d smem=%dB CTAs/SM=%d grid<=%d "
             "(forward%s; unstructured scenes fall back to dual)", C.N, C.NP, cnd::NT, C.smem_bytes, C.ctas_per_sm,
             h->cond_grid, h->dtype == LCPB200_F32 ? "+backward" : "");
  else
    snprintf(cbuf, sizeof(cbuf), "condensed KKT: n/a");
  snprintf(buf, len,
           "dtype=%s n=%d m=%d(pad %d) e=%d | %s | dual: threads=%d smem=%dB T:%s m1=%d ldT=%d ldL=%d G:%s Qinv:%s grid<=%d "
           "ws/CTA=%lldB sms=%d",
           h->dtype == LCPB200_F32 ? "f32" : "f64", P.n, P.m, P.mp, P.e, cbuf, P.nt, P.smem_bytes, modes[P.mode], P.m1,
           P.ldT, P.ldL, P.G_smem ? "smem" : "L2", P.Qi_smem ? "smem" : "L2", h->max_grid,
           (long long)(P.ws_per_cta * (h->dtype == LCPB200_F32 ? 4 : 8)), h->num_sms);
  return 0;
}

template <typename T>
static int launch_forward(lcpb200_handle_s* h, int slot, int B, const void* Q, const void* p, const void* G,
                          const void* hv, const void* A, const void* b, const void* F, double eps,
                          int not_improved_lim, int max_iter, void* zhat, void* nu, void* lam, void* slack,
                          int32_t* status, int32_t* iters, void* resid, void* Rsave, cudaStream_t st,
                          unsigned char* ssave = nullptr) {
  const bool cond = h->cplan.ok != 0;
  if (cond) {
    cnd::CFwdArgs<T> c;
    c.P = h->cplan;
    c.B = B;
    c.Q = (const T*)Q; c.p = (const T*)p; c.G = (const T*)G; c.h = (const T*)hv;
    c.A = (const T*)A; c.b = (const T*)b; c.F = (const T*)F;
    c.zhat = (T*)zhat; c.nu = (T*)nu; c.lam = (T*)lam; c.slack = (T*)slack; c.resid = (T*)resid;
    c.status = status; c.iters = iters;
    c.eps = (T)eps; c.not_improved_lim = not_improved_lim; c.max_iter = max_iter;
    memset(&c.soa, 0, sizeof(c.soa));
    c.ssave = ssave;
    c.prof = h->cprof ? h->cprof + (size_t)slot * h->cond_grid * cnd::CPH_COUNT : nullptr;
    const int cgrid = std::min(B, h->cond_grid);
#define CALL_FWD(NSV) cnd::launch_cond_forward_t<T, NSV>(c, cgrid, st)
    const cudaError_t ce = LCPB200_NS_DISPATCH(h->cplan.NS, CALL_FWD);
#undef CALL_FWD
    CK(ce);
    Rsave = nullptr;
  }
  if (int rc = ensure_ws(h, B)) return rc;
  FwdArgs<T> a;
  a.P = h->plan;
  a.B = B;
  a.Q = (const T*)Q; a.p = (const T*)p; a.G = (const T*)G; a.h = (const T*)hv;
  a.A = (const T*)A; a.b = (const T*)b; a.F = (const T*)F;
  a.zhat = (T*)zhat; a.nu = (T*)nu; a.lam = (T*)lam; a.slack = (T*)slack; a.resid = (T*)resid;
  a.status = status; a.iters = iters;
  a.eps = (T)eps; a.not_improved_lim = not_improved_lim; a.max_iter = max_iter;
  a.Rsave = (T*)Rsave;
  a.fallback_only = cond ? 1 : 0;
  a.ws = (T*)h->ws + (size_t)slot * h->plan.ws_per_cta * h->ws_ctas;
  a.prof = h->prof ? h->prof + (size_t)slot * h->max_grid * PH_COUNT : nullptr;
  const int grid = std::min(B, h->ws_ctas);
  const int mode = h->plan.mode;
  const cudaError_t le = mode == 0   ? launch_forward_t<T, 0>(a, grid, st)
                         : mode == 1 ? launch_forward_t<T, 1>(a, grid, st)
                                     : launch_forward_t<T, 2>(a, grid, st);
  CK(le);
  return 0;
}

template <typename T>
static int launch_backward(lcpb200_handle_s* h, int slot, int B, const void* Q, const void* G, const void* A,
                           const void* F, const void* zhat, const void* nu, const void* lam, const void* slack,
                           const void* g, void* dQ, void* dp, void* dG, void* dh, void* dA, void* db, void* dF,
                           const void* Rsave, unsigned flags, cudaStream_t st, const unsigned char* sload = nullptr) {
  const bool have_cond = h->cplan.ok != 0;
  const bool cond_first = have_cond && sizeof(T) == 4 && !getenv("LCPB200_DUAL_BACKWARD");
  int* flagbuf = nullptr;
  if (have_cond) {
    CK(h->d_flag[slot].ensure(sizeof(int) * (size_t)B));
    flagbuf = (int*)h->d_flag[slot].p;
  }
  cnd::CBwdArgs<T> c;
  if (have_cond) {
    c.P = h->cplan;
    c.B = B;
    c.Q = (const T*)Q; c.G = (const T*)G; c.A = (const T*)A; c.F = (const T*)F;
    c.zhat = (const T*)zhat; c.nu = (const T*)nu; c.lam = (const T*)lam; c.slack = (const T*)slack;
    c.g = (const T*)g;
    c.dQ = (T*)dQ; c.dp = (T*)dp; c.dG = (T*)dG; c.dh = (T*)dh; c.dA = (T*)dA; c.db = (T*)db; c.dF = (T*)dF;
    c.done = cond_first ? flagbuf : nullptr;
    c.only = cond_first ? nullptr : flagbuf;
    c.flags = flags;
    c.sload = sload;
    memset(&c.soa, 0, sizeof(c.soa));
    c.dmass = c.dinertia = c.dv = c.dfext = c.dnormal = c.dp1 = c.dp2 = c.dmu = c.drest = nullptr;
    c.prof = h->cprof ? h->cprof + (size_t)slot * h->cond_grid * cnd::CPH_COUNT : nullptr;
  }
  const int cgrid = std::min(B, std::max(h->cond_grid, 1));
  if (cond_first) {
#define CALL_BWD(NSV) cnd::launch_cond_backward_t<T, NSV>(c, cgrid, st)
    const cudaError_t ce = LCPB200_NS_DISPATCH(h->cplan.NS, CALL_BWD);
#undef CALL_BWD
    CK(ce);
  }
  if (int rc = ensure_ws(h, B)) return rc;
  BwdArgs<T> a;
  a.P = h->plan;
  a.B = B;
  a.Q = (const T*)Q; a.G = (const T*)G; a.A = (const T*)A; a.F = (const T*)F;
  a.zhat = (const T*)zhat; a.nu = (const T*)nu; a.lam = (const T*)lam; a.slack = (const T*)slack;
  a.g = (const T*)g;
  a.dQ = (T*)dQ; a.dp = (T*)dp; a.dG = (T*)dG; a.dh = (T*)dh; a.dA = (T*)dA; a.db = (T*)db; a.dF = (T*)dF;
  a.flags = flags;
  a.Rsave = have_cond ? nullptr : (const T*)Rsave;
  a.skip = cond_first ? flagbuf : nullptr;
  a.bad = (have_cond && !cond_first) ? flagbuf : nullptr;
  a.ws = (T*)h->ws + (size_t)slot * h->plan.ws_per_cta * h->ws_ctas;
  a.prof = h->prof ? h->prof + (size_t)slot * h->max_grid * PH_COUNT : nullptr;
  const int grid = std::min(B, h->ws_ctas);
  const int mode = h->plan.mode;
  const cudaError_t le = mode == 0   ? launch_backward_t<T, 0>(a, grid, st)
                         : mode == 1 ? launch_backward_t<T, 1>(a, grid, st)
                                     : launch_backward_t<T, 2>(a, grid, st);
  CK(le);
  if (have_cond && !cond_first) {
#define CALL_BWD(NSV) cnd::launch_cond_backward_t<T, NSV>(c, cgrid, st)
    const cudaError_t ce = LCPB200_NS_DISPATCH(h->cplan.NS, CALL_BWD);
#undef CALL_BWD
    CK(ce);
  }
  return 0;
}

static int check_fwd_args(lcpb200_handle_t h, int B, const void* Q, const void* p, const void* G, const void* hv,
                          const void* A, const void* b, const void* F, const void* zhat, const void* nu,
                          const void* lam, const void* slack, const void* status, const void* iters,
                          int max_iter) {
  if (!h) return fail("null handle");
  if (B < 0) return fail("B < 0");
  if (!Q || !p || !G || !hv || !F) return fail("Q, p, G, h, F must be non-NULL");
  if (h->e > 0 && (!A || !b)) return fail("handle was created with e > 0 but A or b is NULL");
  if (!zhat || !lam || !slack || !status || !iters) return fail("zhat, lam, slack, status, iters must be non-NULL");
  if (h->e > 0 && !nu) return fail("nu must be non-NULL when e > 0");
  if (max_iter < 0) return fail("max_iter < 0");
  return 0;
}

extern "C" int lcpb200_forward(lcpb200_handle_t h, int B, const void* Q, const void* p, const void* G,
                               const void* hv, const void* A, const void* b, const void* F, double eps,
                               int not_improved_lim, int max_iter, void* zhat, void* nu, void* lam, void* slack,
                               int32_t* status, int32_t* iters, void* resid, void* Rsave, void* stream) {
  if (int rc = check_fwd_args(h, B, Q, p, G, hv, A, b, F, zhat, nu, lam, slack, status, iters, max_iter)) return rc;
  if (!h->dual_ok) return fail("this handle serves the engine entry points only (problem too large for the dense API)");
  if (B == 0) return 0;
  DeviceGuard dg_;
  CK(dg_.set(h->device));
  cudaStream_t st = (cudaStream_t)stream;
  unsigned char* ssave = nullptr;
  h->struct_B = 0;
  if (h->cplan.ok) {
    if ((size_t)B * h->cplan.sbytes > h->d_struct.bytes) CK(cudaDeviceSynchronize());
    CK(h->d_struct.ensure((size_t)B * h->cplan.sbytes));
    ssave = (unsigned char*)h->d_struct.p;
  }
  const int rc = h->dtype == LCPB200_F32
             ? launch_forward<float>(h, 0, B, Q, p, G, hv, A, b, F, eps, not_improved_lim, max_iter, zhat, nu, lam,
                                     slack, status, iters, resid, Rsave, st, ssave)
             : launch_forward<double>(h, 0, B, Q, p, G, hv, A, b, F, eps, not_improved_lim, max_iter, zhat, nu, lam,
                                      slack, status, iters, resid, Rsave, st, ssave);
  if (rc == 0 && ssave) h->struct_B = B;
  return rc;
}

extern "C" int lcpb200_backward(lcpb200_handle_t h, int B, const void* Q, const void* G, const void* A,
                                const void* F, const void* zhat, const void* nu, const void* lam,
                                const void* slack, const void* g, void* dQ, void* dp, void* dG, void* dh, void* dA,
                                void* db, void* dF, const void* Rsave, unsigned flags, void* stream) {
  if (!h) return fail("null handle");
  if (!h->dual_ok) return fail("this handle serves the engine entry points only (problem too large for the dense API)");
  if (B < 0) return fail("B < 0");
  if (!Q || !G || !F || !zhat || !lam || !slack || !g) return fail("Q, G, F, zhat, lam, slack, dl_dzhat must be non-NULL");
  if (h->e > 0 && (!A || !nu)) return fail("A and nu must be non-NULL when e > 0");
  if (flags & ~(LCPB200_BWD_EXACT_ADJOINT | LCPB200_BWD_REUSE_STRUCTURE))
    return fail("flags: LCPB200_BWD_EXACT_ADJOINT | LCPB200_BWD_REUSE_STRUCTURE are the defined bits");
  if (B == 0) return 0;
  DeviceGuard dg_;
  CK(dg_.set(h->device));
  cudaStream_t st = (cudaStream_t)stream;
  const unsigned char* sload = ((flags & LCPB200_BWD_REUSE_STRUCTURE) && h->cplan.ok && h->struct_B == B)
                                   ? (const unsigned char*)h->d_struct.p : nullptr;
  const unsigned kf = flags & LCPB200_BWD_EXACT_ADJOINT;
  return h->dtype == LCPB200_F32
             ? launch_backward<float>(h, 0, B, Q, G, A, F, zhat, nu, lam, slack, g, dQ, dp, dG, dh, dA, db, dF, Rsave, kf, st, sload)
             : launch_backward<double>(h, 0, B, Q, G, A, F, zhat, nu, lam, slack, g, dQ, dp, dG, dh, dA, db, dF, Rsave, kf, st, sload);
}

extern "C" int lcpb200_profile(lcpb200_handle_t h, int enable, long long* out) {
  if (!h) return fail("null handle");
  DeviceGuard dg_;
  CK(dg_.set(h->device));
  const size_t cnt = (size_t)lcpb200_handle_s::NSLOT * h->max_grid * PH_COUNT;
  const size_t ccnt = (size_t)lcpb200_handle_s::NSLOT * std::max(h->cond_grid, h->num_sms) * cnd::CPH_COUNT;
  if (out) {
    for (int i = 0; i < PH_COUNT + cnd::CPH_COUNT; ++i) out[i] = 0;
    if (h->prof) {
      std::vector<long long> tmp(cnt);
      CK(cudaMemcpy(tmp.data(), h->prof, cnt * sizeof(long long), cudaMemcpyDeviceToHost));
      for (size_t i = 0; i < cnt; ++i) out[i % PH_COUNT] += tmp[i];
    }
    if (h->cprof) {
      std::vector<long long> tmp(ccnt);
      CK(cudaMemcpy(tmp.data(), h->cprof, ccnt * sizeof(long long), cudaMemcpyDeviceToHost));
      for (size_t i = 0; i < ccnt; ++i) out[PH_COUNT + i % cnd::CPH_COUNT] += tmp[i];
    }
  }
  if (enable && !h->prof) CK(cudaMalloc(&h->prof, cnt * sizeof(long long)));
  if (enable && !h->cprof) CK(cudaMalloc(&h->cprof, ccnt * sizeof(long long)));
  if (enable) { CK(cudaMemset(h->prof, 0, cnt * sizeof(long long))); CK(cudaMemset(h->cprof, 0, ccnt * sizeof(long long))); }
  if (!enable && h->prof) { cudaFree(h->prof); h->prof = nullptr; }
  if (!enable && h->cprof) { cudaFree(h->cprof); h->cprof = nullptr; }
  return 0;
}

static int ensure_streams(lcpb200_handle_s* h) {
  for (auto& s : h->streams)
    if (!s) CK(cudaStreamCreateWithFlags(&s, cudaStreamNonBlocking));
  return 0;
}

static int chunk_scenes(const lcpb200_handle_s* h, int B) {
  int c = std::max(2 * h->max_grid, (B + 7) / 8);
  return std::max(1, std::min(c, B));
}

extern "C" int lcpb200_forward_host(lcpb200_handle_t h, int B, const void* Q, const void* p, const void* G,
                                    const void* hv, const void* A, const void* b, const void* F, double eps,
                                    int not_improved_lim, int max_iter, void* zhat, void* nu, void* lam,
                                    void* slack, int32_t* status, int32_t* iters, void* resid) {
  if (int rc = check_fwd_args(h, B, Q, p, G, hv, A, b, F, zhat, nu, lam, slack, status, iters, max_iter)) return rc;
  if (!h->dual_ok) return fail("this handle serves the engine entry points only (problem too large for the dense API)");
  if (B == 0) return 0;
  DeviceGuard dg_;
  CK(dg_.set(h->device));
  if (int rc = ensure_streams(h)) return rc;
  const size_t w = h->dtype == LCPB200_F32 ? 4 : 8;
  const size_t n = h->n, m = h->m, e = h->e;
  const size_t in_sz[7] = {n * n * w, n * w, m * n * w, m * w, e * n * w, e * w, m * m * w};
  const void* in_src[7] = {Q, p, G, hv, A, b, F};
  const size_t out_sz[6] = {n * w, e * w, m * w, m * w, 4, 4};
  void* out_dst[6] = {zhat, nu, lam, slack, status, iters};
  for (int i = 0; i < 7; ++i) if (in_sz[i]) CK(h->d_in[i].ensure(in_sz[i] * B));
  for (int i = 0; i < 6; ++i) if (out_sz[i]) CK(h->d_out[i].ensure(out_sz[i] * B));
  DevBuf& d_resid = h->d_bwd[15];
  if (resid) CK(d_resid.ensure(w * B));
  h->retained_B = 0;
  const bool keepR = !h->cplan.ok && (m * m * w * (size_t)B) <= ((size_t)8 << 30);
  if (keepR) CK(h->d_R.ensure(m * m * w * (size_t)B));
  const int C = chunk_scenes(h, B);
  int k = 0;
  for (int s0 = 0; s0 < B; s0 += C, ++k) {
    const int cb = std::min(C, B - s0);
    const int slot = k % lcpb200_handle_s::NSLOT;
    cudaStream_t st = h->streams[slot];
    for (int i = 0; i < 7; ++i)
      if (in_sz[i] && in_src[i])
        CK(cudaMemcpyAsync((char*)h->d_in[i].p + in_sz[i] * s0, (const char*)in_src[i] + in_sz[i] * s0,
                           in_sz[i] * cb, cudaMemcpyHostToDevice, st));
    auto at = [&](DevBuf& bf, size_t per) -> void* { return per ? (char*)bf.p + per * s0 : nullptr; };
    int rc = h->dtype == LCPB200_F32
                 ? launch_forward<float>(h, slot, cb, at(h->d_in[0], in_sz[0]), at(h->d_in[1], in_sz[1]),
                                         at(h->d_in[2], in_sz[2]), at(h->d_in[3], in_sz[3]), at(h->d_in[4], in_sz[4]),
                                         at(h->d_in[5], in_sz[5]), at(h->d_in[6], in_sz[6]), eps, not_improved_lim,
                                         max_iter, at(h->d_out[0], out_sz[0]), at(h->d_out[1], out_sz[1]),
                                         at(h->d_out[2], out_sz[2]), at(h->d_out[3], out_sz[3]),
                                         (int32_t*)at(h->d_out[4], 4), (int32_t*)at(h->d_out[5], 4),
                                         resid ? (char*)d_resid.p + w * s0 : nullptr,
                                         keepR ? (char*)h->d_R.p + m * m * w * s0 : nullptr, st)
                 : launch_forward<double>(h, slot, cb, at(h->d_in[0], in_sz[0]), at(h->d_in[1], in_sz[1]),
                                          at(h->d_in[2], in_sz[2]), at(h->d_in[3], in_sz[3]), at(h->d_in[4], in_sz[4]),
                                          at(h->d_in[5], in_sz[5]), at(h->d_in[6], in_sz[6]), eps, not_improved_lim,
                                          max_iter, at(h->d_out[0], out_sz[0]), at(h->d_out[1], out_sz[1]),
                                          at(h->d_out[2], out_sz[2]), at(h->d_out[3], out_sz[3]),
                                          (int32_t*)at(h->d_out[4], 4), (int32_t*)at(h->d_out[5], 4),
                                          resid ? (char*)d_resid.p + w * s0 : nullptr,
                                          keepR ? (char*)h->d_R.p + m * m * w * s0 : nullptr, st);
    if (rc) return rc;
    for (int i = 0; i < 6; ++i)
      if (out_sz[i] && out_dst[i])
        CK(cudaMemcpyAsync((char*)out_dst[i] + out_sz[i] * s0, (char*)h->d_out[i].p + out_sz[i] * s0,
                           out_sz[i] * cb, cudaMemcpyDeviceToHost, st));
    if (resid)
      CK(cudaMemcpyAsync((char*)resid + w * s0, (char*)d_resid.p + w * s0, w * cb, cudaMemcpyDeviceToHost, st));
  }
  for (auto& s : h->streams) CK(cudaStreamSynchronize(s));
  h->retained_B = B;
  h->retained_R = keepR;
  return 0;
}

extern "C" int lcpb200_backward_host(lcpb200_handle_t h, int B, const void* Q, const void* G, const void* A,
                                     const void* F, const void* zhat, const void* nu, const void* lam,
                                     const void* slack, const void* g, void* dQ, void* dp, void* dG, void* dh,
                                     void* dA, void* db, void* dF, unsigned flags) {
  if (!h) return fail("null handle");
  if (!h->dual_ok) return fail("this handle serves the engine entry points only (problem too large for the dense API)");
  if (B < 0) return fail("B < 0");
  const bool retained = (Q == nullptr);
  if (retained) {
    if (h->retained_B != B || B == 0) return fail("backward_host: no retained forward state for this batch");
    if (!g) return fail("dl_dzhat must be non-NULL");
  } else {
    if (!G || !F || !zhat || !lam || !slack || !g) return fail("Q, G, F, zhat, lam, slack, dl_dzhat must be non-NULL");
    if (h->e > 0 && (!A || !nu)) return fail("A and nu must be non-NULL when e > 0");
  }
  if (flags != LCPB200_BWD_BUG_COMPATIBLE && flags != LCPB200_BWD_EXACT_ADJOINT)
    return fail("flags must be LCPB200_BWD_BUG_COMPATIBLE or LCPB200_BWD_EXACT_ADJOINT");
  if (B == 0) return 0;
  DeviceGuard dg_;
  CK(dg_.set(h->device));
  if (int rc = ensure_streams(h)) return rc;
  const size_t w = h->dtype == LCPB200_F32 ? 4 : 8;
  const size_t n = h->n, m = h->m, e = h->e;
  const size_t in_sz[9] = {n * n * w, m * n * w, e * n * w, m * m * w, n * w, e * w, m * w, m * w, n * w};
  const void* in_src[9] = {Q, G, A, F, zhat, nu, lam, slack, g};
  DevBuf* in_buf[9] = {&h->d_in[0], &h->d_in[2], &h->d_in[4], &h->d_in[6],
                       retained ? &h->d_out[0] : &h->d_bwd[0], retained ? &h->d_out[1] : &h->d_bwd[1],
                       retained ? &h->d_out[2] : &h->d_bwd[2], retained ? &h->d_out[3] : &h->d_bwd[3], &h->d_bwd[4]};
  const bool resident[9] = {retained, retained, retained, retained, retained, retained, retained, retained, false};
  const size_t out_sz[7] = {n * n * w, n * w, m * n * w, m * w, e * n * w, e * w, m * m * w};
  void* out_dst[7] = {dQ, dp, dG, dh, dA, db, dF};
  DevBuf* out_buf[7] = {&h->d_bwd[5], &h->d_bwd[6], &h->d_bwd[7], &h->d_bwd[8], &h->d_bwd[9], &h->d_bwd[10],
                        &h->d_bwd[11]};
  if (!retained) h->retained_B = 0;
  for (int i = 0; i < 9; ++i) if (in_sz[i] && (in_src[i] || resident[i])) CK(in_buf[i]->ensure(in_sz[i] * B));
  for (int i = 0; i < 7; ++i) if (out_sz[i] && out_dst[i]) CK(out_buf[i]->ensure(out_sz[i] * B));
  const int C = chunk_scenes(h, B);
  int k = 0;
  for (int s0 = 0; s0 < B; s0 += C, ++k) {
    const int cb = std::min(C, B - s0);
    const int slot = k % lcpb200_handle_s::NSLOT;
    cudaStream_t st = h->streams[slot];
    for (int i = 0; i < 9; ++i)
      if (in_sz[i] && in_src[i] && !resident[i])
        CK(cudaMemcpyAsync((char*)in_buf[i]->p + in_sz[i] * s0, (const char*)in_src[i] + in_sz[i] * s0,
                           in_sz[i] * cb, cudaMemcpyHostToDevice, st));
    auto ai = [&](int i) -> void* {
      return (in_sz[i] && (in_src[i] || resident[i])) ? (char*)in_buf[i]->p + in_sz[i] * s0 : nullptr;
    };
    const void* rs = (retained && h->retained_R) ? (const char*)h->d_R.p + m * m * w * s0 : nullptr;
    auto ao = [&](int i) -> void* { return (out_sz[i] && out_dst[i]) ? (char*)out_buf[i]->p + out_sz[i] * s0 : nullptr; };
    int rc = h->dtype == LCPB200_F32
                 ? launch_backward<float>(h, slot, cb, ai(0), ai(1), ai(2), ai(3), ai(4), ai(5), ai(6), ai(7), ai(8),
                                          ao(0), ao(1), ao(2), ao(3), ao(4), ao(5), ao(6), rs, flags, st)
                 : launch_backward<double>(h, slot, cb, ai(0), ai(1), ai(2), ai(3), ai(4), ai(5), ai(6), ai(7), ai(8),
                                           ao(0), ao(1), ao(2), ao(3), ao(4), ao(5), ao(6), rs, flags, st);
    if (rc) return rc;
    for (int i = 0; i < 7; ++i)
      if (out_sz[i] && out_dst[i])
        CK(cudaMemcpyAsync((char*)out_dst[i] + out_sz[i] * s0, (char*)out_buf[i]->p + out_sz[i] * s0,
                           out_sz[i] * cb, cudaMemcpyDeviceToHost, st));
  }
  for (auto& s : h->streams) CK(cudaStreamSynchronize(s));
  return 0;
}


template <typename T>
static void fill_soa(cnd::EngineSoA<T>& s, lcpb200_handle_s* h, int B, int nb, int nc, int mode, double dt,
                     const void* mass, const void* inertia, const void* v, const void* fext, const void* normal,
                     const void* p1, const void* p2, const int32_t* b1, const int32_t* b2, const void* mu,
                     const void* rest, const int32_t* nc_s = nullptr) {
  s.mass = (const T*)mass; s.inertia = (const T*)inertia; s.v = (const T*)v; s.fext = (const T*)fext;
  s.normal = (const T*)normal; s.p1 = (const T*)p1; s.p2 = (const T*)p2; s.mu = (const T*)mu; s.rest = (const T*)rest;
  s.b1 = b1; s.b2 = b2; s.nc_s = nc_s; s.nb = nb; s.nc = nc; s.mode = mode; s.dt = (T)dt;
  s.p_s = (T*)h->d_ph.p;
  s.h_s = s.p_s + (size_t)B * h->n;
}

static bool use_banded(const lcpb200_handle_s* h) {
  if (h->dtype != LCPB200_F64) return false;
  return !h->cplan.ok || getenv("LCPB200_FORCE_BANDED") != nullptr;
}

static int ensure_bplan(lcpb200_handle_s* h, int B, int nb, int nc, int mode) {
  if (h->bplan_mode != mode) {
    bnd::BPlan& P = h->bplan;
    memset(&P, 0, sizeof(P));
    P.nb = nb; P.n = h->n; P.ncap = nc; P.cs = mode == 0 ? 4 : 1; P.m = h->m; P.e = h->e;
    if (h->e > bnd::BD) return fail("large-scene kernel: more than 16 equality rows");
    const int dyn_max = h->smem_optin - 1024;
    if (!bnd::carve_bplan(P, dyn_max)) return fail("large-scene kernel: the scene does not fit (shared memory)");
    int occ = 0;
    CK(bnd::configure_band(P.smem_bytes, dyn_max, &occ));
    if (occ < 1) return fail("large-scene kernel cannot be resident");
    P.ok = 1;
    h->bplan_mode = mode;
    h->bws_ctas = 0;
  }
  const int ctas = std::min(B, h->num_sms);
  if (ctas > h->bws_ctas) {
    CK(cudaDeviceSynchronize());
    CK(h->d_bwsd.ensure((size_t)ctas * h->bplan.g_doubles * sizeof(double)));
    CK(h->d_bwsi.ensure((size_t)ctas * h->bplan.i_ints * sizeof(int)));
    h->bws_ctas = ctas;
  }
  return 0;
}

static int check_engine(lcpb200_handle_t h, int B, int nb, int nc, int mode) {
  if (!h) return fail("null handle");
  if (B < 0 || nb <= 0 || nc <= 0) return fail("need B >= 0, nb > 0, nc > 0");
  if (mode != 0 && mode != 1) return fail("mode must be 0 (solve_dynamics) or 1 (post_stabilization)");
  if (!h->cplan.ok && h->dtype != LCPB200_F64)
    return fail("engine entry points: n + e > 128 needs the large-scene kernel, which is fp64 only");
  if (h->n != 3 * nb || h->m != (mode == 0 ? 4 : 1) * nc)
    return fail("handle was created for other sizes: need n = 3 nb and m = 4 nc (mode 0) or nc (mode 1)");
  return 0;
}

template <typename T>
static int engine_forward_t(lcpb200_handle_s* h, int B, int nb, int nc, int mode, double dt, const void* mass,
                            const void* inertia, const void* v, const void* fext, const void* normal, const void* p1,
                            const void* p2, const int32_t* b1, const int32_t* b2, const int32_t* ncs, const void* mu,
                            const void* rest, const void* A, const void* b, double eps, int not_improved_lim, int max_iter, void* zhat,
                            void* nu, void* lam, void* slack, int32_t* status, int32_t* iters, void* resid,
                            cudaStream_t st) {
  CK(h->d_ph.ensure(sizeof(T) * (size_t)B * (h->n + h->m)));
  cnd::CFwdArgs<T> c;
  c.P = h->cplan;
  c.B = B;
  c.Q = nullptr; c.G = nullptr; c.F = nullptr;
  c.A = (const T*)A; c.b = (const T*)b;
  fill_soa<T>(c.soa, h, B, nb, nc, mode, dt, mass, inertia, v, fext, normal, p1, p2, b1, b2, mu, rest, ncs);
  c.ssave = nullptr;
  c.p = c.soa.p_s; c.h = c.soa.h_s;
  c.zhat = (T*)zhat; c.nu = (T*)nu; c.lam = (T*)lam; c.slack = (T*)slack; c.resid = (T*)resid;
  c.status = status; c.iters = iters;
  c.eps = (T)eps; c.not_improved_lim = not_improved_lim; c.max_iter = max_iter;
  c.prof = h->cprof;
  const int cgrid = std::min(B, h->cond_grid);
#define CALL_FWD(NSV) cnd::launch_cond_forward_t<T, NSV>(c, cgrid, st)
  const cudaError_t ce = LCPB200_NS_DISPATCH(h->cplan.NS, CALL_FWD);
#undef CALL_FWD
  CK(ce);
  return 0;
}

extern "C" int lcpb200_engine_forward(lcpb200_handle_t h, int B, int nb, int nc, int mode, double dt,
                                      const void* mass, const void* inertia, const void* v, const void* fext,
                                      const void* normal, const void* p1, const void* p2, const int32_t* body1,
                                      const int32_t* body2, const int32_t* contact_count, const void* mu,
                                      const void* restitution, const void* A, const void* b, double eps, int not_improved_lim, int max_iter, void* zhat,
                                      void* nu, void* lam, void* slack, int32_t* status, int32_t* iters, void* resid,
                                      void* stream) {
  if (int rc = check_engine(h, B, nb, nc, mode)) return rc;
  if (!mass || !inertia || !v || !normal || !p1 || !p2 || !body1 || !body2 || !restitution) return fail("engine_forward: NULL input");
  if (mode == 0 && (!fext || !mu)) return fail("engine_forward: fext and mu are needed for mode 0");
  if (h->e > 0 && (!A || !b || !nu)) return fail("handle was created with e > 0 but A, b or nu is NULL");
  if (!zhat || !lam || !slack || !status || !iters) return fail("zhat, lam, slack, status, iters must be non-NULL");
  if (B == 0) return 0;
  DeviceGuard dg_;
  CK(dg_.set(h->device));
  cudaStream_t st = (cudaStream_t)stream;
  if (use_banded(h)) {
    if (int rc = ensure_bplan(h, B, nb, nc, mode)) return rc;
    bnd::BArgs a;
    a.P = h->bplan;
    a.B = B;
    memset(&a.soa, 0, sizeof(a.soa));
    a.soa.mass = (const double*)mass; a.soa.inertia = (const double*)inertia; a.soa.v = (const double*)v;
    a.soa.fext = (const double*)fext; a.soa.normal = (const double*)normal; a.soa.p1 = (const double*)p1;
    a.soa.p2 = (const double*)p2; a.soa.mu = (const double*)mu; a.soa.rest = (const double*)restitution;
    a.soa.b1 = body1; a.soa.b2 = body2; a.soa.nc_s = contact_count; a.soa.nb = nb; a.soa.nc = nc; a.soa.mode = mode;
    a.soa.dt = dt;
    a.A = (const double*)A; a.b = (const double*)b;
    a.zhat = (double*)zhat; a.nu = (double*)nu; a.lam = (double*)lam; a.slack = (double*)slack; a.resid = (double*)resid;
    a.status = status; a.iters = iters;
    a.eps = eps; a.not_improved_lim = not_improved_lim; a.max_iter = max_iter;
    a.wsd = (double*)h->d_bwsd.p; a.wsi = (int*)h->d_bwsi.p;
    a.prof = h->cprof;
    CK(bnd::launch_band_forward(a, std::min(B, h->num_sms), st));
    return 0;
  }
  return h->dtype == LCPB200_F32
             ? engine_forward_t<float>(h, B, nb, nc, mode, dt, mass, inertia, v, fext, normal, p1, p2, body1, body2,
                                       contact_count, mu, restitution, A, b, eps, not_improved_lim, max_iter, zhat, nu, lam, slack, status,
                                       iters, resid, st)
             : engine_forward_t<double>(h, B, nb, nc, mode, dt, mass, inertia, v, fext, normal, p1, p2, body1, body2,
                                        contact_count, mu, restitution, A, b, eps, not_improved_lim, max_iter, zhat, nu, lam, slack, status,
                                        iters, resid, st);
}

template <typename T>
static int engine_backward_t(lcpb200_handle_s* h, int B, int nb, int nc, int mode, double dt, const void* mass,
                             const void* inertia, const void* v, const void* fext, const void* normal, const void* p1,
                             const void* p2, const int32_t* b1, const int32_t* b2, const int32_t* ncs, const void* mu,
                             const void* rest, const void* A, const void* zhat, const void* nu, const void* lam, const void* slack,
                             const void* g, void* dmass, void* dinertia, void* dv, void* dfext, void* dnormal,
                             void* dp1, void* dp2, void* dmu, void* drest, void* dA, void* db, unsigned flags,
                             cudaStream_t st) {
  CK(h->d_ph.ensure(sizeof(T) * (size_t)B * (h->n + h->m)));
  cnd::CBwdArgs<T> c;
  c.P = h->cplan;
  c.B = B;
  c.Q = nullptr; c.G = nullptr; c.F = nullptr; c.A = (const T*)A;
  c.zhat = (const T*)zhat; c.nu = (const T*)nu; c.lam = (const T*)lam; c.slack = (const T*)slack; c.g = (const T*)g;
  c.dQ = c.dp = c.dG = c.dh = c.dF = nullptr;
  c.dA = (T*)dA; c.db = (T*)db;
  c.done = nullptr; c.only = nullptr; c.flags = flags; c.sload = nullptr;
  c.prof = h->cprof;
  fill_soa<T>(c.soa, h, B, nb, nc, mode, dt, mass, inertia, v, fext, normal, p1, p2, b1, b2, mu, rest, ncs);
  c.dmass = (T*)dmass; c.dinertia = (T*)dinertia; c.dv = (T*)dv; c.dfext = (T*)dfext; c.dnormal = (T*)dnormal;
  c.dp1 = (T*)dp1; c.dp2 = (T*)dp2; c.dmu = (T*)dmu; c.drest = (T*)drest;
  const int cgrid = std::min(B, h->cond_grid);
#define CALL_BWD(NSV) cnd::launch_cond_backward_t<T, NSV>(c, cgrid, st)
  const cudaError_t ce = LCPB200_NS_DISPATCH(h->cplan.NS, CALL_BWD);
#undef CALL_BWD
  CK(ce);
  return 0;
}

extern "C" int lcpb200_engine_backward(lcpb200_handle_t h, int B, int nb, int nc, int mode, double dt,
                                       const void* mass, const void* inertia, const void* v, const void* fext,
                                       const void* normal, const void* p1, const void* p2, const int32_t* body1,
                                       const int32_t* body2, const int32_t* contact_count, const void* mu,
                                       const void* restitution, const void* A, const void* zhat, const void* nu, const void* lam, const void* slack,
                                       const void* dl_dzhat, void* dmass, void* dinertia, void* dv, void* dfext,
                                       void* dnormal, void* dp1, void* dp2, void* dmu, void* drestitution, void* dA,
                                       void* db, unsigned flags, void* stream) {
  if (int rc = check_engine(h, B, nb, nc, mode)) return rc;
  if (!mass || !inertia || !v || !normal || !p1 || !p2 || !body1 || !body2 || !restitution) return fail("engine_backward: NULL input");
  if (mode == 0 && !mu) return fail("engine_backward: mu is needed for mode 0");
  if (!zhat || !lam || !slack || !dl_dzhat) return fail("zhat, lam, slack, dl_dzhat must be non-NULL");
  if (h->e > 0 && (!A || !nu)) return fail("A and nu must be non-NULL when e > 0");
  if (flags != LCPB200_BWD_BUG_COMPATIBLE && flags != LCPB200_BWD_EXACT_ADJOINT)
    return fail("flags must be LCPB200_BWD_BUG_COMPATIBLE or LCPB200_BWD_EXACT_ADJOINT");
  if (B == 0) return 0;
  DeviceGuard dg_;
  CK(dg_.set(h->device));
  cudaStream_t st = (cudaStream_t)stream;
  if (use_banded(h)) {
    if (int rc = ensure_bplan(h, B, nb, nc, mode)) return rc;
    bnd::BBwdArgs a;
    a.P = h->bplan;
    a.B = B;
    memset(&a.soa, 0, sizeof(a.soa));
    a.soa.mass = (const double*)mass; a.soa.inertia = (const double*)inertia; a.soa.v = (const double*)v;
    a.soa.fext = (const double*)fext; a.soa.normal = (const double*)normal; a.soa.p1 = (const double*)p1;
    a.soa.p2 = (const double*)p2; a.soa.mu = (const double*)mu; a.soa.rest = (const double*)restitution;
    a.soa.b1 = body1; a.soa.b2 = body2; a.soa.nc_s = contact_count; a.soa.nb = nb; a.soa.nc = nc; a.soa.mode = mode;
    a.soa.dt = dt;
    a.A = (const double*)A;
    a.zhat = (const double*)zhat; a.nu = (const double*)nu; a.lam = (const double*)lam; a.slack = (const double*)slack;
    a.g = (const double*)dl_dzhat;
    a.dmass = (double*)dmass; a.dinertia = (double*)dinertia; a.dv = (double*)dv; a.dfext = (double*)dfext;
    a.dnormal = (double*)dnormal; a.dp1 = (double*)dp1; a.dp2 = (double*)dp2; a.dmu = (double*)dmu;
    a.drest = (double*)drestitution; a.dA = (double*)dA; a.db = (double*)db;
    a.wsd = (double*)h->d_bwsd.p; a.wsi = (int*)h->d_bwsi.p;
    a.prof = h->cprof;
    a.flags = flags;
    CK(bnd::launch_band_backward(a, std::min(B, h->num_sms), st));
    return 0;
  }
  return h->dtype == LCPB200_F32
             ? engine_backward_t<float>(h, B, nb, nc, mode, dt, mass, inertia, v, fext, normal, p1, p2, body1, body2,
                                        contact_count, mu, restitution, A, zhat, nu, lam, slack, dl_dzhat, dmass, dinertia, dv, dfext,
                                        dnormal, dp1, dp2, dmu, drestitution, dA, db, flags, st)
             : engine_backward_t<double>(h, B, nb, nc, mode, dt, mass, inertia, v, fext, normal, p1, p2, body1, body2,
                                         contact_count, mu, restitution, A, zhat, nu, lam, slack, dl_dzhat, dmass, dinertia, dv, dfext,
                                         dnormal, dp1, dp2, dmu, drestitution, dA, db, flags, st);
}

extern "C" int lcpb200_find_contacts(int dtype, int B, int nb, int cap, double eps, const void* pos, const void* rad,
                                     int32_t* body1, int32_t* body2, int32_t* counts, void* stream) {
  if (dtype != LCPB200_F32 && dtype != LCPB200_F64) return fail("bad dtype");
  if (B < 0 || nb <= 0 || cap <= 0) return fail("find_contacts: need B >= 0, nb > 0, cap > 0");
  if (!pos || !rad || !body1 || !body2 || !counts) return fail("find_contacts: NULL argument");
  if (B == 0) return 0;
  int dev = 0, sms = 0;
  CK(cudaGetDevice(&dev));
  CK(cudaDeviceGetAttribute(&sms, cudaDevAttrMultiProcessorCount, dev));
  cudaStream_t st = (cudaStream_t)stream;
  if (dtype == LCPB200_F32)
    cts::launch_find_contacts<float>(B, nb, cap, (float)eps, (const float*)pos, (const float*)rad, body1, body2, counts, sms, st);
  else
    cts::launch_find_contacts<double>(B, nb, cap, eps, (const double*)pos, (const double*)rad, body1, body2, counts, sms, st);
  CK(cudaGetLastError());
  return 0;
}

extern "C" int lcpb200_contact_geometry(int dtype, int B, int nb, int cap, const void* pos, const void* rad,
                                        const void* fric, const void* rest, const int32_t* body1, const int32_t* body2,
                                        const int32_t* counts, void* normal, void* p1, void* p2, void* pen, void* mu,
                                        void* rest_c, void* stream) {
  if (dtype != LCPB200_F32 && dtype != LCPB200_F64) return fail("bad dtype");
  if (B < 0 || nb <= 0 || cap <= 0) return fail("contact_geometry: need B >= 0, nb > 0, cap > 0");
  if (!pos || !rad || !fric || !rest || !body1 || !body2 || !counts || !normal || !p1 || !p2 || !pen || !mu || !rest_c)
    return fail("contact_geometry: NULL argument");
  if (B == 0) return 0;
  int dev = 0, sms = 0;
  CK(cudaGetDevice(&dev));
  CK(cudaDeviceGetAttribute(&sms, cudaDevAttrMultiProcessorCount, dev));
  cudaStream_t st = (cudaStream_t)stream;
  if (dtype == LCPB200_F32)
    cts::launch_contact_geometry<float>(B, nb, cap, (const float*)pos, (const float*)rad, (const float*)fric,
                                        (const float*)rest, body1, body2, counts, (float*)normal, (float*)p1, (float*)p2,
                                        (float*)pen, (float*)mu, (float*)rest_c, sms, st);
  else
    cts::launch_contact_geometry<double>(B, nb, cap, (const double*)pos, (const double*)rad, (const double*)fric,
                                         (const double*)rest, body1, body2, counts, (double*)normal, (double*)p1,
                                         (double*)p2, (double*)pen, (double*)mu, (double*)rest_c, sms, st);
  CK(cudaGetLastError());
  return 0;
}

extern "C" int lcpb200_assemble(int dtype, int B, int nb, int nc, double dt, const void* mass, const void* inertia,
                                const void* v, const void* fext, const void* normal, const void* p1,
                                const void* p2, const int32_t* body1, const int32_t* body2, const void* mu,
                                const void* restitution, void* Q, void* p, void* G, void* hv, void* F,
                                void* stream) {
  if (dtype != LCPB200_F32 && dtype != LCPB200_F64) return fail("bad dtype");
  if (B < 0 || nb <= 0 || nc <= 0) return fail("need B >= 0, nb > 0, nc > 0");
  if (!mass || !inertia || !v || !fext || !normal || !p1 || !p2 || !body1 || !body2 || !mu || !restitution)
    return fail("assemble: NULL input");
  if (!Q || !p || !G || !hv || !F) return fail("assemble: NULL output");
  if (B == 0) return 0;
  cudaStream_t st = (cudaStream_t)stream;
  if (dtype == LCPB200_F32)
    launch_assemble<float>(B, nb, nc, (float)dt, (const float*)mass, (const float*)inertia, (const float*)v,
                           (const float*)fext, (const float*)normal, (const float*)p1, (const float*)p2, body1,
                           body2, (const float*)mu, (const float*)restitution, (float*)Q, (float*)p, (float*)G,
                           (float*)hv, (float*)F, st);
  else
    launch_assemble<double>(B, nb, nc, dt, (const double*)mass, (const double*)inertia, (const double*)v,
                            (const double*)fext, (const double*)normal, (const double*)p1, (const double*)p2,
                            body1, body2, (const double*)mu, (const double*)restitution, (double*)Q, (double*)p,
                            (double*)G, (double*)hv, (double*)F, st);
  CK(cudaGetLastError());
  return 0;
}

extern "C" int lcpb200_assemble_backward(int dtype, int B, int nb, int nc, double dt, const void* mass,
                                         const void* inertia, const void* v, const void* normal, const void* p1,
                                         const void* p2, const int32_t* body1, const int32_t* body2,
                                         const void* mu, const void* restitution, const void* dQ, const void* dp,
                                         const void* dG, const void* dh, const void* dF, void* dmass,
                                         void* dinertia, void* dv, void* dfext, void* dnormal, void* dp1,
                                         void* dp2, void* dmu, void* drestitution, void* stream) {
  if (dtype != LCPB200_F32 && dtype != LCPB200_F64) return fail("bad dtype");
  if (B < 0 || nb <= 0 || nc <= 0) return fail("need B >= 0, nb > 0, nc > 0");
  if (!mass || !inertia || !v || !normal || !p1 || !p2 || !body1 || !body2 || !mu || !restitution)
    return fail("assemble_backward: NULL input");
  if (!dQ || !dp || !dG || !dh || !dF) return fail("assemble_backward: NULL upstream gradient");
  if (B == 0) return 0;
  cudaStream_t st = (cudaStream_t)stream;
  if (dtype == LCPB200_F32)
    launch_assemble_backward<float>(B, nb, nc, (float)dt, (const float*)mass, (const float*)inertia,
                                    (const float*)v, (const float*)normal, (const float*)p1, (const float*)p2,
                                    body1, body2, (const float*)mu, (const float*)restitution, (const float*)dQ,
                                    (const float*)dp, (const float*)dG, (const float*)dh, (const float*)dF,
                                    (float*)dmass, (float*)dinertia, (float*)dv, (float*)dfext, (float*)dnormal,
                                    (float*)dp1, (float*)dp2, (float*)dmu, (float*)drestitution, st);
  else
    launch_assemble_backward<double>(B, nb, nc, dt, (const double*)mass, (const double*)inertia, (const double*)v,
                                     (const double*)normal, (const double*)p1, (const double*)p2, body1, body2,
                                     (const double*)mu, (const double*)restitution, (const double*)dQ,
                                     (const double*)dp, (const double*)dG, (const double*)dh, (const double*)dF,
                                     (double*)dmass, (double*)dinertia, (double*)dv, (double*)dfext,
                                     (double*)dnormal, (double*)dp1, (double*)dp2, (double*)dmu,
                                     (double*)drestitution, st);
  CK(cudaGetLastError());
  return 0;
}
```

### lcp_physics_b200/lcp.py

```python
import ctypes

import torch

from . import _lib

SINGULAR_Q_MSG = """
lcp Error: Cannot perform LU factorization on Q.
Please make sure that your Q matrix is PSD and has
a non-zero diagonal.
"""

INACCURATE_MSG = """
--------
lcp warning: Returning an inaccurate and potentially incorrect solution.
Some residual is large; the problem may be infeasible or difficult.
Try verbose output and more iterations (max_iter).
--------
"""


def _sizes(Q, p, G, h, A, b, F):
    if G.dim() != 3:
        raise ValueError("G must be [B, nineq, nz]")
    B, m, n = G.shape
    e = A.shape[1] if A.dim() > 1 else 0
    if not (e > 0 or m > 0):
        raise AssertionError("need neq > 0 or nineq > 0")
    if m == 0:
        raise ValueError("lcp_physics_b200 needs at least one inequality row (the reference crashes on nineq == 0)")
    exp = {"Q": (B, n, n), "p": (B, n), "h": (B, m), "F": (B, m, m)}
    for name, t in (("Q", Q), ("p", p), ("h", h), ("F", F)):
        if tuple(t.shape) != exp[name]:
            raise ValueError("%s has shape %s, expected %s" % (name, tuple(t.shape), exp[name]))
    if e > 0 and (tuple(A.shape) != (B, e, n) or tuple(b.shape) != (B, e)):
        raise ValueError("A/b have shapes %s/%s, expected %s/%s"
                         % (tuple(A.shape), tuple(b.shape), (B, e, n), (B, e)))
    return B, n, m, e


def _stream_ptr(device):
    return ctypes.c_void_p(torch.cuda.current_stream(device).cuda_stream)


def solve_forward(Q, p, G, h, A, b, F, eps=1e-12, not_improved_lim=3, max_iter=10, out=None, save=None):
    _lib.require_cuda()
    lib = _lib.load()
    B, n, m, e = _sizes(Q, p, G, h, A, b, F)
    dtype, dev = Q.dtype, Q.device
    ins = [t.contiguous() for t in (Q, p, G, h)] + \
          [A.contiguous() if e > 0 else None, b.contiguous() if e > 0 else None, F.contiguous()]
    for t in ins:
        if t is not None and (t.dtype != dtype or t.device != dev):
            raise ValueError("all LCP inputs must share dtype and device")
    on_host = dev.type != "cuda"
    dev_index = torch.cuda.current_device() if on_host else dev.index
    hd = _lib.get_handle(dtype, n, m, e, dev_index,
                         "host" if on_host else torch.cuda.current_stream(dev).cuda_stream)
    if out is not None:
        zhat, nu, lam, slack, status, iters, resid = out
    else:
        mk = lambda *shape, dt=dtype: torch.empty(*shape, dtype=dt, device=dev)
        zhat, lam, slack = mk(B, n), mk(B, m), mk(B, m)
        nu = mk(B, e) if e > 0 else None
        status = mk(B, dt=torch.int32)
        iters = mk(B, dt=torch.int32)
        resid = mk(B)
    if B == 0:
        return zhat, nu, lam, slack, status, iters, resid
    args = [hd.raw, B] + [_lib.ptr(t) for t in ins] + [float(eps), int(not_improved_lim), int(max_iter)] + \
           [_lib.ptr(t) for t in (zhat, nu, lam, slack, status, iters, resid)]
    if on_host:
        hd.host_generation += 1
        _lib.check(lib.lcpb200_forward_host(*args))
        if save is not None:
            save["token"] = (hd, hd.host_generation, B)
    else:
        hd.fwd_generation += 1
        with torch.cuda.device(dev):
            _lib.check(lib.lcpb200_forward(*args, None, _stream_ptr(dev)))
        if save is not None:
            save["struct"] = (hd, hd.fwd_generation, B)
    return zhat, nu, lam, slack, status, iters, resid


def solve_backward(Q, G, A, F, zhat, nu, lam, slack, dl_dzhat, need=(True,) * 7, out=None, saved=None,
                   exact_adjoint=False):
    _lib.require_cuda()
    lib = _lib.load()
    B, m, n = G.shape
    e = A.shape[1] if (A is not None and A.dim() > 1) else 0
    dtype, dev = G.dtype, G.device
    on_host = dev.type != "cuda"
    dev_index = torch.cuda.current_device() if on_host else dev.index
    hd = _lib.get_handle(dtype, n, m, e, dev_index,
                         "host" if on_host else torch.cuda.current_stream(dev).cuda_stream)
    mk = lambda *shape: torch.empty(*shape, dtype=dtype, device=dev)
    shapes = [(B, n, n), (B, n), (B, m, n), (B, m), (B, e, n), (B, e), (B, m, m)]
    outs = []
    for k, shp in enumerate(shapes):
        want = need[k] and not (k in (4, 5) and e == 0)
        if out is not None:
            outs.append(out[k] if want else None)
        else:
            outs.append(mk(*shp) if want else None)
    if B == 0:
        return tuple(outs)
    ins = [Q.contiguous(), G.contiguous(), A.contiguous() if e > 0 else None, F.contiguous(),
           zhat.contiguous(), nu.contiguous() if e > 0 else None, lam.contiguous(), slack.contiguous(),
           dl_dzhat.contiguous().to(dtype)]
    if on_host:
        tok = saved.get("token") if saved else None
        if tok is not None and tok[0] is hd and tok[1] == hd.host_generation and tok[2] == B:
            in_ptrs = [None] * 8 + [_lib.ptr(ins[8])]
        else:
            in_ptrs = [_lib.ptr(t) for t in ins]
        hd.host_generation += 1
        _lib.check(lib.lcpb200_backward_host(hd.raw, B, *in_ptrs, *[_lib.ptr(t) for t in outs], 1 if exact_adjoint else 0))
    else:
        tok = saved.get("struct") if saved else None
        reuse = tok is not None and tok[0] is hd and tok[1] == hd.fwd_generation and tok[2] == B
        flags = (1 if exact_adjoint else 0) | (2 if reuse else 0)
        args = [hd.raw, B] + [_lib.ptr(t) for t in ins] + [_lib.ptr(t) for t in outs] + [None, flags]
        with torch.cuda.device(dev):
            _lib.check(lib.lcpb200_backward(*args, _stream_ptr(dev)))
    return tuple(outs)


class _LCPFn(torch.autograd.Function):
    @staticmethod
    def forward(ctx, Q, p, G, h, A, b, F, opts):
        need_bwd = any(ctx.needs_input_grad[:7])
        ctx.saved_state = {} if need_bwd else None
        zhat, nu, lam, slack, status, iters, resid = solve_forward(
            Q, p, G, h, A, b, F, opts.eps, opts.not_improved_lim, opts.max_iter, save=ctx.saved_state)
        if bool((status == _lib.STATUS_SINGULAR_Q).any()):
            raise RuntimeError(SINGULAR_Q_MSG)
        if opts.verbose >= 0 and bool((resid > 1.0).any()):
            print(INACCURATE_MSG)
            print(resid.max())
        e = A.shape[1] if A.dim() > 1 else 0
        ctx.e = e
        ctx.exact_adjoint = bool(getattr(opts, "exact_adjoint", False))
        ctx.save_for_backward(zhat, Q, G, A if e > 0 else None, F, nu, lam, slack)
        ctx.AB_proto = (A, b)
        opts.nus, opts.lams, opts.slacks = nu, lam, slack
        opts.status, opts.iters, opts.resids = status, iters, resid
        return zhat

    @staticmethod
    def backward(ctx, dl_dzhat):
        zhat, Q, G, A, F, nu, lam, slack = ctx.saved_tensors
        need = list(ctx.needs_input_grad[:7])
        dQ, dp, dG, dh, dA, db, dF = solve_backward(Q, G, A, F, zhat, nu, lam, slack, dl_dzhat, need,
                                                    saved=ctx.saved_state, exact_adjoint=ctx.exact_adjoint)
        return dQ, dp, dG, dh, dA, db, dF, None


class LCPFunction:

    def __init__(self, eps=1e-12, verbose=-1, not_improved_lim=3, max_iter=10, exact_adjoint=False):
        self.exact_adjoint = exact_adjoint
        self.eps = eps
        self.verbose = verbose
        self.not_improved_lim = not_improved_lim
        self.max_iter = max_iter
        self.nus = self.lams = self.slacks = None
        self.status = self.iters = self.resids = None

    def __call__(self, Q, p, G, h, A, b, F):
        return _LCPFn.apply(Q, p, G, h, A, b, F, self)
```

Measured before the change: 305,800.

## Split structure scan into separate higher-occupancy kernel before condensed solves

Moves the sparsity-structure scan of Q/G/A/F out of the condensed forward and backward kernels into a dedicated structure kernel. That kernel uses a smaller shared-memory plan and runs at 3 CTAs per SM, then saves the result to a global buffer that the solve kernels reload. The solve kernels' shared-memory K region shrinks because it no longer needs the full scan scratch, which may raise their occupancy. The cost is an extra kernel launch, a global round trip of the structure data, and new per-slot structure buffers. The L2 prefetches are also removed.

New measurement: 312,900 (median of 6 runs). +2.3%, better.

```diff
diff --git a/lcp_physics_b200/csrc/lcp_cond_kernels.cu b/lcp_physics_b200/csrc/lcp_cond_kernels.cu
--- a/lcp_physics_b200/csrc/lcp_cond_kernels.cu
+++ b/lcp_physics_b200/csrc/lcp_cond_kernels.cu
@@ -31,5 +31,19 @@
   return cudaSuccess;
 }
 
+template <>
+cudaError_t launch_cond_structure_t<LCP_T, LCP_NS>(const CStructArgs<LCP_T>& a, int grid, cudaStream_t st) {
+  cond_structure_kernel<LCP_T, LCP_NS><<<grid, NT, a.P.smem_bytes, st>>>(a);
+  return cudaGetLastError();
+}
+
+template <>
+cudaError_t configure_cond_structure_t<LCP_T, LCP_NS>(int smem_bytes, int dyn_max, int* occ) {
+  const void* f = (const void*)cond_structure_kernel<LCP_T, LCP_NS>;
+  cudaError_t e;
+  if ((e = cudaFuncSetAttribute(f, cudaFuncAttributeMaxDynamicSharedMemorySize, dyn_max)) != cudaSuccess) return e;
+  return cudaOccupancyMaxActiveBlocksPerMultiprocessor(occ, f, NT, smem_bytes);
+}
+
 }
 }
diff --git a/lcp_physics_b200/csrc/lcp_cond_launch.h b/lcp_physics_b200/csrc/lcp_cond_launch.h
--- a/lcp_physics_b200/csrc/lcp_cond_launch.h
+++ b/lcp_physics_b200/csrc/lcp_cond_launch.h
@@ -8,6 +8,8 @@
 template <typename T, int NS> cudaError_t launch_cond_forward_t(const CFwdArgs<T>& a, int grid, cudaStream_t st);
 template <typename T, int NS> cudaError_t launch_cond_backward_t(const CBwdArgs<T>& a, int grid, cudaStream_t st);
 template <typename T, int NS> cudaError_t configure_cond_t(int smem_bytes, int dyn_max, int* occ);
+template <typename T, int NS> cudaError_t launch_cond_structure_t(const CStructArgs<T>& a, int grid, cudaStream_t st);
+template <typename T, int NS> cudaError_t configure_cond_structure_t(int smem_bytes, int dyn_max, int* occ);
 
 }
 }
diff --git a/lcp_physics_b200/csrc/lcp_condensed.cuh b/lcp_physics_b200/csrc/lcp_condensed.cuh
--- a/lcp_physics_b200/csrc/lcp_condensed.cuh
+++ b/lcp_physics_b200/csrc/lcp_condensed.cuh
@@ -13,6 +13,8 @@
 constexpr int MISC_BAND_LU = 4;
 constexpr int CFLAG_DENSE_LU = 4;
 constexpr int STATUS_UNSUPPORTED = -100;
+constexpr int STRUCT_UNSUPPORTED = -1;
+constexpr int STRUCT_SINGULAR = -2;
 
 struct CPlan {
   int ok;
@@ -32,13 +34,14 @@
   return al16((size_t)2 * KS * m * 2) + al16((size_t)2 * KS * m * tsize) + al16((size_t)5 * m * 4) +
          al16((size_t)CSMAX * m * 2) + al16((size_t)8 * m * 4) + al16((size_t)LMAX * n * 2) + al16((size_t)n * 4) + 64;
 }
+__host__ __device__ inline size_t soa_scratch_bytes(int n) { return al16((size_t)LMAX * n * 2) + al16((size_t)n * 4); }
 
 inline size_t carve_plan(CPlan& P, int tsize) {
   size_t o = 0;
   const int n = P.n, m = P.m, e = P.e, NP = P.NP, pcap = P.pcap, wcap = P.wcap;
 #define CND_TAKE(field, bytes) do { P.field = (int)o; o += al16((size_t)(bytes)); } while (0)
   size_t kb = (size_t)NP * NP * 8;
-  if (scratch_bytes(n, m, tsize) > kb) kb = scratch_bytes(n, m, tsize);
+  if (soa_scratch_bytes(n) > kb) kb = soa_scratch_bytes(n);
   if ((size_t)8 * NP * 8 > kb) kb = (size_t)8 * NP * 8;
   { const size_t qn = (NP + 31) / 32, sl = (size_t)(NP / qn) * qn * qn * 32 * 8; if (sl > kb) kb = sl; }
   CND_TAKE(o_K, kb);
@@ -66,6 +69,23 @@
   return o;
 }
 
+inline size_t carve_struct_plan(const CPlan& P, CPlan& S, int tsize) {
+  S = P;
+  size_t o = al16(scratch_bytes(P.n, P.m, tsize));
+  S.o_K = 0;
+  const int d1 = (int)o - P.o_Fd;
+  o += P.o_x - P.o_Fd;
+  S.o_Fd += d1; S.o_Gd += d1; S.o_As += d1; S.o_x += d1;
+  const int d2 = (int)o - P.o_qd;
+  o += P.o_y - P.o_qd;
+  S.o_qd += d2; S.o_y += d2;
+  const int d3 = (int)o - P.o_rows;
+  o += P.o_misc - P.o_rows + 16 * 4;
+  S.o_rows += d3; S.o_posof += d3; S.o_clist += d3; S.o_ccols += d3; S.o_ncols += d3; S.o_clcnt += d3; S.o_misc += d3;
+  S.smem_bytes = (int)o;
+  return o;
+}
+
 extern __shared__ __align__(16) unsigned char cnd_smem[];
 
 template <typename T>
@@ -169,20 +189,11 @@
   return bad;
 }
 
-__device__ __forceinline__ void prefetch_l2(const void* p, size_t bytes) {
-  const char* c = reinterpret_cast<const char*>(p);
-  for (size_t o = (size_t)threadIdx.x * 128; o < bytes; o += (size_t)NT * 128)
-    asm volatile("prefetch.global.L2 [%0];" ::"l"(c + o));
-}
-
 template <typename T>
 __device__ __noinline__ bool build_structure(const CPlan& P, CSmem<T>& S, Struct& st, const T* __restrict__ Q,
                                              const T* __restrict__ G, const T* __restrict__ A,
                                              const T* __restrict__ F, int* singular) {
   const int n = P.n, m = P.m, e = P.e, tid = threadIdx.x, lane = tid & 31, warp = tid >> 5, pcap = P.pcap;
-  prefetch_l2(F, (size_t)m * m * sizeof(T));
-  prefetch_l2(G, (size_t)m * n * sizeof(T));
-  prefetch_l2(Q, (size_t)n * n * sizeof(T));
   char* sb = reinterpret_cast<char*>(S.K());
   unsigned short* Fi = reinterpret_cast<unsigned short*>(sb);
   unsigned short* Gi = Fi + (size_t)KS * m;
@@ -948,21 +959,21 @@
 struct CFwdArgs {
   CPlan P;
   int B;
-  const T *Q, *p, *G, *h, *A, *b, *F;
+  const T *p, *h, *A, *b;
   T *zhat, *nu, *lam, *slack, *resid;
   int *status, *iters;
   T eps;
   int not_improved_lim, max_iter;
   long long* prof;
   EngineSoA<T> soa;
-  unsigned char* ssave;
+  const unsigned char* sload;
 };
 
 template <typename T>
 struct CBwdArgs {
   CPlan P;
   int B;
-  const T *Q, *G, *A, *F;
+  const T* A;
   const T *zhat, *nu, *lam, *slack, *g;
   T *dQ, *dp, *dG, *dh, *dA, *db, *dF;
   int* done;
@@ -980,8 +991,9 @@
   for (int i = threadIdx.x; i < (bytes >> 4); i += NT) d4[i] = s4[i];
 }
 
-__device__ __forceinline__ void save_structure(const CPlan& P, const Struct& st, bool ok, unsigned char* dst) {
-  if (threadIdx.x == 0) *reinterpret_cast<int4*>(dst) = make_int4(ok ? st.ncomp : -1, st.cs, st.sh, st.m);
+__device__ __forceinline__ void save_structure(const CPlan& P, const Struct& st, int code, unsigned char* dst) {
+  const bool ok = code == 0;
+  if (threadIdx.x == 0) *reinterpret_cast<int4*>(dst) = make_int4(ok ? st.ncomp : code, st.cs, st.sh, st.m);
   if (!ok) return;
   const int c1 = P.o_x - P.o_Fd, c2 = P.o_y - P.o_qd, c3 = P.o_misc - P.o_rows;
   copy16(dst + 16, cnd_smem + P.o_Fd, c1);
@@ -998,6 +1010,35 @@
   copy16(cnd_smem + P.o_qd, src + 16 + c1, c2);
   copy16(cnd_smem + P.o_rows, src + 16 + c1 + c2, c3);
   return true;
+}
+
+template <typename T>
+struct CStructArgs {
+  CPlan P;
+  int B;
+  const T *Q, *G, *A, *F;
+  const int* only;
+  unsigned char* ssave;
+};
+
+constexpr int STRUCT_CTAS = 3;
+template <typename T, int NS>
+__global__ void __launch_bounds__(NT, STRUCT_CTAS) cond_structure_kernel(const __grid_constant__ CStructArgs<T> a) {
+  const CPlan& P = a.P;
+  CSmem<T> S(P);
+  const int n = P.n, m = P.m, e = P.e, tid = threadIdx.x;
+  __shared__ int singular_s;
+  for (int sc = blockIdx.x; sc < a.B; sc += gridDim.x) {
+    if (a.only && !a.only[sc]) continue;
+    if (tid == 0) singular_s = 0;
+    __syncthreads();
+    Struct st;
+    const bool ok = build_structure<T>(P, S, st, a.Q + (size_t)sc * n * n, a.G + (size_t)sc * m * n,
+                                       e > 0 ? a.A + (size_t)sc * e * n : nullptr, a.F + (size_t)sc * m * m, &singular_s);
+    __syncthreads();
+    save_structure(P, st, ok ? 0 : (singular_s ? STRUCT_SINGULAR : STRUCT_UNSUPPORTED), a.ssave + (size_t)sc * P.sbytes);
+    __syncthreads();
+  }
 }
 
 template <typename T>
@@ -1179,13 +1220,11 @@
     Struct st;
     const bool ok = a.soa.mass
         ? build_structure_soa<T>(P, S, st, a.soa, sc, e > 0 ? a.A + (size_t)sc * e * n : nullptr, &singular_s)
-        : build_structure<T>(P, S, st, a.Q + (size_t)sc * n * n, a.G + (size_t)sc * m * n,
-                             e > 0 ? a.A + (size_t)sc * e * n : nullptr, a.F + (size_t)sc * m * m, &singular_s);
-    __syncthreads();
-    if (a.ssave) save_structure(P, st, ok, a.ssave + (size_t)sc * P.sbytes);
+        : load_structure(P, st, a.sload + (size_t)sc * P.sbytes);
+    __syncthreads();
     pf.lap(CPH_STRUCT);
     if (!ok) {
-      if (singular_s) {
+      if (a.soa.mass ? singular_s != 0 : st.ncomp == STRUCT_SINGULAR) {
         for (int i = tid; i < n; i += NT) a.zhat[(size_t)sc * n + i] = NANV;
         for (int i = tid; i < m; i += NT) { a.lam[(size_t)sc * m + i] = NANV; a.slack[(size_t)sc * m + i] = NANV; }
         for (int i = tid; i < e; i += NT) a.nu[(size_t)sc * e + i] = NANV;
@@ -1375,7 +1414,7 @@
 __global__ void __launch_bounds__(NT, (NS <= 6) ? 2 : 1) cond_backward_kernel(const __grid_constant__ CBwdArgs<T> a) {
   const CPlan& P = a.P;
   CSmem<T> S(P);
-  const int n = P.n, m = P.m, e = P.e, tid = threadIdx.x;
+  const int n = P.n, e = P.e, tid = threadIdx.x;
   __shared__ int singular_s;
   Prof<PROF> pf(PROF ? a.prof + (size_t)blockIdx.x * CPH_COUNT : nullptr);
   for (int sc = blockIdx.x; sc < a.B; sc += gridDim.x) {
@@ -1386,10 +1425,7 @@
     Struct st;
     const bool ok = a.soa.mass
         ? build_structure_soa<T>(P, S, st, a.soa, sc, e > 0 ? a.A + (size_t)sc * e * n : nullptr, &singular_s)
-        : a.sload
-              ? load_structure(P, st, a.sload + (size_t)sc * P.sbytes)
-              : build_structure<T>(P, S, st, a.Q + (size_t)sc * n * n, a.G + (size_t)sc * m * n,
-                                   e > 0 ? a.A + (size_t)sc * e * n : nullptr, a.F + (size_t)sc * m * m, &singular_s);
+        : load_structure(P, st, a.sload + (size_t)sc * P.sbytes);
     __syncthreads();
     pf.lap(CPH_STRUCT);
     if (!ok) {
diff --git a/lcp_physics_b200/csrc/lcpb200.cu b/lcp_physics_b200/csrc/lcpb200.cu
--- a/lcp_physics_b200/csrc/lcpb200.cu
+++ b/lcp_physics_b200/csrc/lcpb200.cu
@@ -59,6 +59,8 @@
   int max_grid;
   CPlan cplan;
   int cond_grid = 0;
+  CPlan splan;
+  int struct_grid = 0;
   static const int NSLOT = 2;
   void* ws = nullptr;
   size_t ws_bytes = 0;
@@ -76,6 +78,7 @@
   long long* cprof = nullptr;
   DevBuf d_struct;
   int struct_B = 0;
+  DevBuf d_hstruct[NSLOT];
   DevBuf d_R;
   int retained_B = 0;
   bool retained_R = false;
@@ -195,7 +198,9 @@
     for (int mult = cnd::CSMAX; mult >= 1; --mult) {
       C.wcap = mult * C.pcap;
       const size_t bytes = cnd::carve_plan(C, (int)sizeof(T));
-      if ((long long)bytes <= lim) { best = (int)bytes; break; }
+      CPlan S;
+      const size_t sbytes = cnd::carve_struct_plan(C, S, (int)sizeof(T));
+      if ((long long)bytes <= lim && (long long)sbytes <= dyn_max) { best = (int)bytes; break; }
       if (mult <= 4) break;
     }
   }
@@ -207,9 +212,19 @@
 #undef CALL_CFG
   if (ce != cudaSuccess) return fail(std::string("condensed kernel configuration: ") + cudaGetErrorString(ce));
   if (occ < 1) return 0;
+  cnd::carve_struct_plan(C, h->splan, (int)sizeof(T));
+  int socc = 0;
+#define CALL_SCFG(NSV) cnd::configure_cond_structure_t<T, NSV>(h->splan.smem_bytes, dyn_max, &socc)
+  const cudaError_t se = LCPB200_NS_DISPATCH(NS, CALL_SCFG);
+#undef CALL_SCFG
+  if (se != cudaSuccess) return fail(std::string("structure kernel configuration: ") + cudaGetErrorString(se));
+  if (socc < 1) return 0;
+  h->struct_grid = socc * h->num_sms;
+  h->splan.ctas_per_sm = socc;
   C.ctas_per_sm = occ;
   h->cond_grid = occ * h->num_sms;
   C.ok = 1;
+  h->splan.ok = 1;
   return 0;
 }
 
@@ -265,6 +280,7 @@
   dg_.set(h->device);
   if (h->ws) cudaFree(h->ws);
   h->d_struct.release();
+  for (auto& b : h->d_hstruct) b.release();
   if (h->prof) cudaFree(h->prof);
   if (h->cprof) cudaFree(h->cprof);
   for (auto& s : h->streams) if (s) cudaStreamDestroy(s);
@@ -290,8 +306,9 @@
   char cbuf[256];
   if (C.ok)
     snprintf(cbuf, sizeof(cbuf), "condensed KKT: N=%d(pad %d) fp64 LU in registers, threads=%d smem=%dB CTAs/SM=%d grid<=%d "
-             "(forward%s; unstructured scenes fall back to dual)", C.N, C.NP, cnd::NT, C.smem_bytes, C.ctas_per_sm,
-             h->cond_grid, h->dtype == LCPB200_F32 ? "+backward" : "");
+             "(forward%s; unstructured scenes fall back to dual); structure scan smem=%dB CTAs/SM=%d", C.N, C.NP, cnd::NT,
+             C.smem_bytes, C.ctas_per_sm, h->cond_grid, h->dtype == LCPB200_F32 ? "+backward" : "", h->splan.smem_bytes,
+             h->splan.ctas_per_sm);
   else
     snprintf(cbuf, sizeof(cbuf), "condensed KKT: n/a");
   snprintf(buf, len,
@@ -304,23 +321,41 @@
 }
 
 template <typename T>
+static int launch_structure(lcpb200_handle_s* h, int B, const void* Q, const void* G, const void* A, const void* F,
+                            const int* only, unsigned char* sbuf, cudaStream_t st) {
+  cnd::CStructArgs<T> s;
+  s.P = h->splan;
+  s.B = B;
+  s.Q = (const T*)Q; s.G = (const T*)G; s.A = (const T*)A; s.F = (const T*)F;
+  s.only = only;
+  s.ssave = sbuf;
+  const int grid = std::min(B, h->struct_grid);
+#define CALL_STRUCT(NSV) cnd::launch_cond_structure_t<T, NSV>(s, grid, st)
+  const cudaError_t ce = LCPB200_NS_DISPATCH(h->cplan.NS, CALL_STRUCT);
+#undef CALL_STRUCT
+  CK(ce);
+  return 0;
+}
+
+template <typename T>
 static int launch_forward(lcpb200_handle_s* h, int slot, int B, const void* Q, const void* p, const void* G,
                           const void* hv, const void* A, const void* b, const void* F, double eps,
                           int not_improved_lim, int max_iter, void* zhat, void* nu, void* lam, void* slack,
                           int32_t* status, int32_t* iters, void* resid, void* Rsave, cudaStream_t st,
-                          unsigned char* ssave = nullptr) {
+                          unsigned char* sbuf) {
   const bool cond = h->cplan.ok != 0;
   if (cond) {
+    if (int rc = launch_structure<T>(h, B, Q, G, A, F, nullptr, sbuf, st)) return rc;
     cnd::CFwdArgs<T> c;
     c.P = h->cplan;
     c.B = B;
-    c.Q = (const T*)Q; c.p = (const T*)p; c.G = (const T*)G; c.h = (const T*)hv;
-    c.A = (const T*)A; c.b = (const T*)b; c.F = (const T*)F;
+    c.p = (const T*)p; c.h = (const T*)hv;
+    c.A = (const T*)A; c.b = (const T*)b;
     c.zhat = (T*)zhat; c.nu = (T*)nu; c.lam = (T*)lam; c.slack = (T*)slack; c.resid = (T*)resid;
     c.status = status; c.iters = iters;
     c.eps = (T)eps; c.not_improved_lim = not_improved_lim; c.max_iter = max_iter;
     memset(&c.soa, 0, sizeof(c.soa));
-    c.ssave = ssave;
+    c.sload = sbuf;
     c.prof = h->cprof ? h->cprof + (size_t)slot * h->cond_grid * cnd::CPH_COUNT : nullptr;
     const int cgrid = std::min(B, h->cond_grid);
 #define CALL_FWD(NSV) cnd::launch_cond_forward_t<T, NSV>(c, cgrid, st)
@@ -355,7 +390,8 @@
 static int launch_backward(lcpb200_handle_s* h, int slot, int B, const void* Q, const void* G, const void* A,
                            const void* F, const void* zhat, const void* nu, const void* lam, const void* slack,
                            const void* g, void* dQ, void* dp, void* dG, void* dh, void* dA, void* db, void* dF,
-                           const void* Rsave, unsigned flags, cudaStream_t st, const unsigned char* sload = nullptr) {
+                           const void* Rsave, unsigned flags, cudaStream_t st, const unsigned char* sload,
+                           unsigned char* sbuf) {
   const bool have_cond = h->cplan.ok != 0;
   const bool cond_first = have_cond && sizeof(T) == 4 && !getenv("LCPB200_DUAL_BACKWARD");
   int* flagbuf = nullptr;
@@ -367,20 +403,22 @@
   if (have_cond) {
     c.P = h->cplan;
     c.B = B;
-    c.Q = (const T*)Q; c.G = (const T*)G; c.A = (const T*)A; c.F = (const T*)F;
+    c.A = (const T*)A;
     c.zhat = (const T*)zhat; c.nu = (const T*)nu; c.lam = (const T*)lam; c.slack = (const T*)slack;
     c.g = (const T*)g;
     c.dQ = (T*)dQ; c.dp = (T*)dp; c.dG = (T*)dG; c.dh = (T*)dh; c.dA = (T*)dA; c.db = (T*)db; c.dF = (T*)dF;
     c.done = cond_first ? flagbuf : nullptr;
     c.only = cond_first ? nullptr : flagbuf;
     c.flags = flags;
-    c.sload = sload;
+    c.sload = sload ? sload : sbuf;
     memset(&c.soa, 0, sizeof(c.soa));
     c.dmass = c.dinertia = c.dv = c.dfext = c.dnormal = c.dp1 = c.dp2 = c.dmu = c.drest = nullptr;
     c.prof = h->cprof ? h->cprof + (size_t)slot * h->cond_grid * cnd::CPH_COUNT : nullptr;
   }
   const int cgrid = std::min(B, std::max(h->cond_grid, 1));
   if (cond_first) {
+    if (!sload)
+      if (int rc = launch_structure<T>(h, B, Q, G, A, F, nullptr, sbuf, st)) return rc;
 #define CALL_BWD(NSV) cnd::launch_cond_backward_t<T, NSV>(c, cgrid, st)
     const cudaError_t ce = LCPB200_NS_DISPATCH(h->cplan.NS, CALL_BWD);
 #undef CALL_BWD
@@ -407,6 +445,8 @@
                                      : launch_backward_t<T, 2>(a, grid, st);
   CK(le);
   if (have_cond && !cond_first) {
+    if (!sload)
+      if (int rc = launch_structure<T>(h, B, Q, G, A, F, flagbuf, sbuf, st)) return rc;
 #define CALL_BWD(NSV) cnd::launch_cond_backward_t<T, NSV>(c, cgrid, st)
     const cudaError_t ce = LCPB200_NS_DISPATCH(h->cplan.NS, CALL_BWD);
 #undef CALL_BWD
@@ -470,12 +510,19 @@
   DeviceGuard dg_;
   CK(dg_.set(h->device));
   cudaStream_t st = (cudaStream_t)stream;
-  const unsigned char* sload = ((flags & LCPB200_BWD_REUSE_STRUCTURE) && h->cplan.ok && h->struct_B == B)
-                                   ? (const unsigned char*)h->d_struct.p : nullptr;
+  const bool reuse = (flags & LCPB200_BWD_REUSE_STRUCTURE) && h->cplan.ok && h->struct_B == B;
+  const unsigned char* sload = reuse ? (const unsigned char*)h->d_struct.p : nullptr;
+  unsigned char* sbuf = nullptr;
+  if (h->cplan.ok && !reuse) {
+    if ((size_t)B * h->cplan.sbytes > h->d_struct.bytes) CK(cudaDeviceSynchronize());
+    CK(h->d_struct.ensure((size_t)B * h->cplan.sbytes));
+    sbuf = (unsigned char*)h->d_struct.p;
+    h->struct_B = 0;
+  }
   const unsigned kf = flags & LCPB200_BWD_EXACT_ADJOINT;
   return h->dtype == LCPB200_F32
-             ? launch_backward<float>(h, 0, B, Q, G, A, F, zhat, nu, lam, slack, g, dQ, dp, dG, dh, dA, db, dF, Rsave, kf, st, sload)
-             : launch_backward<double>(h, 0, B, Q, G, A, F, zhat, nu, lam, slack, g, dQ, dp, dG, dh, dA, db, dF, Rsave, kf, st, sload);
+             ? launch_backward<float>(h, 0, B, Q, G, A, F, zhat, nu, lam, slack, g, dQ, dp, dG, dh, dA, db, dF, Rsave, kf, st, sload, sbuf)
+             : launch_backward<double>(h, 0, B, Q, G, A, F, zhat, nu, lam, slack, g, dQ, dp, dG, dh, dA, db, dF, Rsave, kf, st, sload, sbuf);
 }
 
 extern "C" int lcpb200_profile(lcpb200_handle_t h, int enable, long long* out) {
@@ -514,6 +561,12 @@
 static int chunk_scenes(const lcpb200_handle_s* h, int B) {
   int c = std::max(2 * h->max_grid, (B + 7) / 8);
   return std::max(1, std::min(c, B));
+}
+
+static int ensure_chunk_structs(lcpb200_handle_s* h, int C) {
+  if (!h->cplan.ok) return 0;
+  for (auto& b : h->d_hstruct) CK(b.ensure((size_t)C * h->cplan.sbytes));
+  return 0;
 }
 
 extern "C" int lcpb200_forward_host(lcpb200_handle_t h, int B, const void* Q, const void* p, const void* G,
@@ -540,11 +593,13 @@
   const bool keepR = !h->cplan.ok && (m * m * w * (size_t)B) <= ((size_t)8 << 30);
   if (keepR) CK(h->d_R.ensure(m * m * w * (size_t)B));
   const int C = chunk_scenes(h, B);
+  if (int rc = ensure_chunk_structs(h, C)) return rc;
   int k = 0;
   for (int s0 = 0; s0 < B; s0 += C, ++k) {
     const int cb = std::min(C, B - s0);
     const int slot = k % lcpb200_handle_s::NSLOT;
     cudaStream_t st = h->streams[slot];
+    unsigned char* sbuf = (unsigned char*)h->d_hstruct[slot].p;
     for (int i = 0; i < 7; ++i)
       if (in_sz[i] && in_src[i])
         CK(cudaMemcpyAsync((char*)h->d_in[i].p + in_sz[i] * s0, (const char*)in_src[i] + in_sz[i] * s0,
@@ -558,7 +613,7 @@
                                          at(h->d_out[2], out_sz[2]), at(h->d_out[3], out_sz[3]),
                                          (int32_t*)at(h->d_out[4], 4), (int32_t*)at(h->d_out[5], 4),
                                          resid ? (char*)d_resid.p + w * s0 : nullptr,
-                                         keepR ? (char*)h->d_R.p + m * m * w * s0 : nullptr, st)
+                                         keepR ? (char*)h->d_R.p + m * m * w * s0 : nullptr, st, sbuf)
                  : launch_forward<double>(h, slot, cb, at(h->d_in[0], in_sz[0]), at(h->d_in[1], in_sz[1]),
                                           at(h->d_in[2], in_sz[2]), at(h->d_in[3], in_sz[3]), at(h->d_in[4], in_sz[4]),
                                           at(h->d_in[5], in_sz[5]), at(h->d_in[6], in_sz[6]), eps, not_improved_lim,
@@ -566,7 +621,7 @@
                                           at(h->d_out[2], out_sz[2]), at(h->d_out[3], out_sz[3]),
                                           (int32_t*)at(h->d_out[4], 4), (int32_t*)at(h->d_out[5], 4),
                                           resid ? (char*)d_resid.p + w * s0 : nullptr,
-                                          keepR ? (char*)h->d_R.p + m * m * w * s0 : nullptr, st);
+                                          keepR ? (char*)h->d_R.p + m * m * w * s0 : nullptr, st, sbuf);
     if (rc) return rc;
     for (int i = 0; i < 6; ++i)
       if (out_sz[i] && out_dst[i])
@@ -618,11 +673,13 @@
   for (int i = 0; i < 9; ++i) if (in_sz[i] && (in_src[i] || resident[i])) CK(in_buf[i]->ensure(in_sz[i] * B));
   for (int i = 0; i < 7; ++i) if (out_sz[i] && out_dst[i]) CK(out_buf[i]->ensure(out_sz[i] * B));
   const int C = chunk_scenes(h, B);
+  if (int rc = ensure_chunk_structs(h, C)) return rc;
   int k = 0;
   for (int s0 = 0; s0 < B; s0 += C, ++k) {
     const int cb = std::min(C, B - s0);
     const int slot = k % lcpb200_handle_s::NSLOT;
     cudaStream_t st = h->streams[slot];
+    unsigned char* sbuf = (unsigned char*)h->d_hstruct[slot].p;
     for (int i = 0; i < 9; ++i)
       if (in_sz[i] && in_src[i] && !resident[i])
         CK(cudaMemcpyAsync((char*)in_buf[i]->p + in_sz[i] * s0, (const char*)in_src[i] + in_sz[i] * s0,
@@ -634,9 +691,9 @@
     auto ao = [&](int i) -> void* { return (out_sz[i] && out_dst[i]) ? (char*)out_buf[i]->p + out_sz[i] * s0 : nullptr; };
     int rc = h->dtype == LCPB200_F32
                  ? launch_backward<float>(h, slot, cb, ai(0), ai(1), ai(2), ai(3), ai(4), ai(5), ai(6), ai(7), ai(8),
-                                          ao(0), ao(1), ao(2), ao(3), ao(4), ao(5), ao(6), rs, flags, st)
+                                          ao(0), ao(1), ao(2), ao(3), ao(4), ao(5), ao(6), rs, flags, st, nullptr, sbuf)
                  : launch_backward<double>(h, slot, cb, ai(0), ai(1), ai(2), ai(3), ai(4), ai(5), ai(6), ai(7), ai(8),
-                                           ao(0), ao(1), ao(2), ao(3), ao(4), ao(5), ao(6), rs, flags, st);
+                                           ao(0), ao(1), ao(2), ao(3), ao(4), ao(5), ao(6), rs, flags, st, nullptr, sbuf);
     if (rc) return rc;
     for (int i = 0; i < 7; ++i)
       if (out_sz[i] && out_dst[i])
@@ -712,10 +769,9 @@
   cnd::CFwdArgs<T> c;
   c.P = h->cplan;
   c.B = B;
-  c.Q = nullptr; c.G = nullptr; c.F = nullptr;
   c.A = (const T*)A; c.b = (const T*)b;
   fill_soa<T>(c.soa, h, B, nb, nc, mode, dt, mass, inertia, v, fext, normal, p1, p2, b1, b2, mu, rest, ncs);
-  c.ssave = nullptr;
+  c.sload = nullptr;
   c.p = c.soa.p_s; c.h = c.soa.h_s;
   c.zhat = (T*)zhat; c.nu = (T*)nu; c.lam = (T*)lam; c.slack = (T*)slack; c.resid = (T*)resid;
   c.status = status; c.iters = iters;
@@ -786,7 +842,7 @@
   cnd::CBwdArgs<T> c;
   c.P = h->cplan;
   c.B = B;
-  c.Q = nullptr; c.G = nullptr; c.F = nullptr; c.A = (const T*)A;
+  c.A = (const T*)A;
   c.zhat = (const T*)zhat; c.nu = (const T*)nu; c.lam = (const T*)lam; c.slack = (const T*)slack; c.g = (const T*)g;
   c.dQ = c.dp = c.dG = c.dh = c.dF = nullptr;
   c.dA = (T*)dA; c.db = (T*)db;
diff --git a/lcp_physics_b200/lcp.py b/lcp_physics_b200/lcp.py
--- a/lcp_physics_b200/lcp.py
+++ b/lcp_physics_b200/lcp.py
@@ -120,6 +120,8 @@
         tok = saved.get("struct") if saved else None
         reuse = tok is not None and tok[0] is hd and tok[1] == hd.fwd_generation and tok[2] == B
         flags = (1 if exact_adjoint else 0) | (2 if reuse else 0)
+        if not reuse:
+            hd.fwd_generation += 1
         args = [hd.raw, B] + [_lib.ptr(t) for t in ins] + [_lib.ptr(t) for t in outs] + [None, flags]
         with torch.cuda.device(dev):
             _lib.check(lib.lcpb200_backward(*args, _stream_ptr(dev)))
```
